# iwa-shi/CRDR

Measured on AMD Instinct MI355X. Metric: stage-3 training img/s at 256x256, higher is better.
Workload: dtype fp32; 1 GPU; config/crdr_stage_3.yaml -b 16: full GAN step (G + 5x CLIC21GVAE D + LPIPS-Alex, random-init weights), rate index cycled 0..4; global_batch=16, crop=256, parallelism=dp1

## Files before the change

crdr_amd/csrc/algo_id.hpp:

```cpp
#pragma once

namespace crdr {

enum AlgoFamily { kAlgoBuiltIn, kAlgoTiled , kAlgoStream, kAlgoWino2, kAlgoWino4, kAlgoBeyond  };
struct AlgoId {
  AlgoFamily family;
  int index;
  int split;
};

inline AlgoId algo_decode(int id, const int (&sizes)[4]) {
  const int base = id & 0xff, split = (id >> 8) & 0xf;
  for (int f = 0, first = 1; id != 0 && f < 4; first += sizes[f++])
    if (base >= first && base < first + sizes[f]) return {AlgoFamily(kAlgoTiled + f), base - first, split};
  return {id == 0 ? kAlgoBuiltIn : kAlgoBeyond, base - 1, split};
}
inline AlgoId conv_algo_decode(int reserved, int ntiled, int nstream) { return algo_decode(reserved, {ntiled, nstream, 2, 1}); }
inline AlgoId wgrad_algo_decode(int algo, int ndirect) { return algo_decode(algo & 0xffff, {ndirect, 0, 1, 1}); }

inline int conv_algo_splits(const AlgoId& id) { return id.family == kAlgoWino4 ? id.split + 1 : 1 << id.split; }
inline int wgrad_algo_splits(const AlgoId& id) { return 1 << id.split; }

inline int conv_algo_encode(AlgoFamily family, int index, int nsplit, int ntiled, int nstream) {
  const int first[] = {1, 1 + ntiled, 1 + ntiled + nstream, 1 + ntiled + nstream + 2};
  int ls = 0;
  while ((1 << ls) < nsplit) ++ls;
  return (first[family - kAlgoTiled] + index) | ((family == kAlgoWino4 ? nsplit - 1 : ls) << 8);
}

}
```

crdr_amd/csrc/api.cpp:

```cpp
#include <hip/hip_runtime.h>
#include <stdarg.h>
#include <stdio.h>

#include <mutex>
#include <vector>

#include "crdr_hip.h"

namespace crdr {
static thread_local char g_err[512] = "";
void set_error(const char* fmt, ...) {
  va_list ap;
  va_start(ap, fmt);
  vsnprintf(g_err, sizeof(g_err), fmt, ap);
  va_end(ap);
}
}

namespace crdr {
struct ProfRec { int kind; double flops; hipEvent_t e0, e1; };
static std::mutex g_pm;
static std::vector<ProfRec> g_recs;
static bool g_prof = false;
bool profile_on() { return g_prof; }
void* profile_begin(hipStream_t s) {
  if (!g_prof) return nullptr;
  hipEvent_t* ev = new hipEvent_t[2];
  if (hipEventCreate(&ev[0]) != hipSuccess || hipEventCreate(&ev[1]) != hipSuccess) { delete[] ev; return nullptr; }
  (void)hipEventRecord(ev[0], s);
  return ev;
}
void profile_end(int kind, double flops, void* token, hipStream_t s) {
  if (!token) return;
  hipEvent_t* ev = static_cast<hipEvent_t*>(token);
  (void)hipEventRecord(ev[1], s);
  std::lock_guard<std::mutex> lk(g_pm);
  g_recs.push_back({kind, flops, ev[0], ev[1]});
  delete[] ev;
}
}

extern "C" void crdr_profile_enable(int on) {
  std::lock_guard<std::mutex> lk(crdr::g_pm);
  crdr::g_prof = on != 0;
}
extern "C" int crdr_profile_read(int kind, double* flops, double* ms, long long* launches) {
  std::lock_guard<std::mutex> lk(crdr::g_pm);
  double f = 0, t = 0;
  long long n = 0;
  std::vector<crdr::ProfRec> keep;
  for (auto& r : crdr::g_recs) {
    if (r.kind != kind) { keep.push_back(r); continue; }
    (void)hipEventSynchronize(r.e1);
    float dt = 0.f;
    if (hipEventElapsedTime(&dt, r.e0, r.e1) == hipSuccess) { f += r.flops; t += dt; ++n; }
    (void)hipEventDestroy(r.e0);
    (void)hipEventDestroy(r.e1);
  }
  crdr::g_recs.swap(keep);
  if (flops) *flops = f;
  if (ms) *ms = t;
  if (launches) *launches = n;
  return 0;
}

extern "C" const char* crdr_last_error(void) { return crdr::g_err; }
extern "C" int crdr_version(void) { return 600; }
extern "C" const char* crdr_arch(void) { return "gfx950"; }
```

crdr_amd/csrc/igemm.hip:

```cpp
#include <algorithm>
#include <type_traits>

#include "algo_id.hpp"
#include "igemm_kernel.hpp"
#include "wino.hpp"

namespace crdr {

extern template __global__ void igemm_kernel<4, 1, 1, 1, false, 0, false>(const IgemmArgs, const IgemmTaps, const IgemmGroup);
extern template __global__ void igemm_kernel<4, 1, 1, 2, false, 0, false>(const IgemmArgs, const IgemmTaps, const IgemmGroup);
extern template __global__ void igemm_kernel<4, 1, 1, 3, false, 0, false>(const IgemmArgs, const IgemmTaps, const IgemmGroup);
extern template __global__ void igemm_kernel<4, 1, 1, 4, false, 0, false>(const IgemmArgs, const IgemmTaps, const IgemmGroup);
extern template __global__ void igemm_kernel<4, 1, 1, 5, false, 0, false>(const IgemmArgs, const IgemmTaps, const IgemmGroup);
extern template __global__ void igemm_kernel<4, 1, 1, 6, false, 0, false>(const IgemmArgs, const IgemmTaps, const IgemmGroup);
extern template __global__ void igemm_kernel<4, 1, 1, 7, false, 0, false>(const IgemmArgs, const IgemmTaps, const IgemmGroup);
extern template __global__ void igemm_kernel<4, 1, 2, 2, false, 0, false>(const IgemmArgs, const IgemmTaps, const IgemmGroup);
extern template __global__ void igemm_kernel<4, 1, 2, 3, false, 0, false>(const IgemmArgs, const IgemmTaps, const IgemmGroup);
extern template __global__ void igemm_kernel<4, 1, 2, 4, false, 0, false>(const IgemmArgs, const IgemmTaps, const IgemmGroup);
extern template __global__ void igemm_kernel<2, 2, 2, 2, false, 0, false>(const IgemmArgs, const IgemmTaps, const IgemmGroup);
extern template __global__ void igemm_kernel<2, 2, 1, 1, false, 0, false>(const IgemmArgs, const IgemmTaps, const IgemmGroup);
extern template __global__ void igemm_kernel<2, 2, 1, 2, false, 0, false>(const IgemmArgs, const IgemmTaps, const IgemmGroup);
extern template __global__ void igemm_kernel<2, 2, 1, 3, false, 0, false>(const IgemmArgs, const IgemmTaps, const IgemmGroup);
extern template __global__ void igemm_kernel<2, 2, 1, 4, false, 0, false>(const IgemmArgs, const IgemmTaps, const IgemmGroup);
extern template __global__ void igemm_kernel<1, 4, 1, 1, false, 0, false>(const IgemmArgs, const IgemmTaps, const IgemmGroup);
extern template __global__ void igemm_kernel<1, 4, 1, 2, false, 0, false>(const IgemmArgs, const IgemmTaps, const IgemmGroup);
extern template __global__ void igemm_kernel<4, 2, 1, 1, false, 0, false>(const IgemmArgs, const IgemmTaps, const IgemmGroup);
extern template __global__ void igemm_kernel<4, 2, 1, 2, false, 0, false>(const IgemmArgs, const IgemmTaps, const IgemmGroup);
extern template __global__ void igemm_kernel<4, 2, 1, 3, false, 0, false>(const IgemmArgs, const IgemmTaps, const IgemmGroup);
extern template __global__ void igemm_kernel<4, 2, 2, 1, false, 0, false>(const IgemmArgs, const IgemmTaps, const IgemmGroup);
extern template __global__ void igemm_kernel<4, 2, 2, 2, false, 0, false>(const IgemmArgs, const IgemmTaps, const IgemmGroup);
extern template __global__ void igemm_kernel<2, 4, 1, 1, false, 0, false>(const IgemmArgs, const IgemmTaps, const IgemmGroup);
extern template __global__ void igemm_kernel<2, 4, 2, 1, false, 0, false>(const IgemmArgs, const IgemmTaps, const IgemmGroup);
extern template __global__ void igemm_kernel<2, 4, 1, 2, false, 0, false>(const IgemmArgs, const IgemmTaps, const IgemmGroup);
extern template __global__ void igemm_kernel<2, 2, 2, 1, false, 0, false>(const IgemmArgs, const IgemmTaps, const IgemmGroup);
extern template __global__ void igemm_kernel<2, 2, 2, 3, false, 0, false>(const IgemmArgs, const IgemmTaps, const IgemmGroup);
extern template __global__ void igemm_kernel<4, 1, 1, 1, true, 0, false>(const IgemmArgs, const IgemmTaps, const IgemmGroup);
extern template __global__ void igemm_kernel<4, 1, 1, 2, true, 0, false>(const IgemmArgs, const IgemmTaps, const IgemmGroup);
extern template __global__ void igemm_kernel<4, 1, 2, 2, true, 0, false>(const IgemmArgs, const IgemmTaps, const IgemmGroup);
extern template __global__ void igemm_kernel<2, 2, 2, 2, true, 0, false>(const IgemmArgs, const IgemmTaps, const IgemmGroup);
extern template __global__ void igemm_kernel<4, 2, 1, 1, true, 0, false>(const IgemmArgs, const IgemmTaps, const IgemmGroup);
extern template __global__ void igemm_kernel<4, 2, 1, 2, true, 0, false>(const IgemmArgs, const IgemmTaps, const IgemmGroup);
extern template __global__ void igemm_kernel<4, 2, 2, 1, true, 0, false>(const IgemmArgs, const IgemmTaps, const IgemmGroup);
extern template __global__ void igemm_kernel<4, 2, 2, 2, true, 0, false>(const IgemmArgs, const IgemmTaps, const IgemmGroup);
extern template __global__ void igemm_kernel<2, 4, 2, 1, true, 0, false>(const IgemmArgs, const IgemmTaps, const IgemmGroup);
extern template __global__ void igemm_kernel<4, 1, 1, 1, false, 3, false>(const IgemmArgs, const IgemmTaps, const IgemmGroup);
extern template __global__ void igemm_kernel<4, 1, 1, 2, false, 3, false>(const IgemmArgs, const IgemmTaps, const IgemmGroup);
extern template __global__ void igemm_kernel<4, 1, 1, 3, false, 3, false>(const IgemmArgs, const IgemmTaps, const IgemmGroup);
extern template __global__ void igemm_kernel<4, 1, 1, 4, false, 3, false>(const IgemmArgs, const IgemmTaps, const IgemmGroup);
extern template __global__ void igemm_kernel<4, 1, 1, 5, false, 3, false>(const IgemmArgs, const IgemmTaps, const IgemmGroup);
extern template __global__ void igemm_kernel<4, 1, 1, 6, false, 3, false>(const IgemmArgs, const IgemmTaps, const IgemmGroup);
extern template __global__ void igemm_kernel<4, 1, 1, 7, false, 3, false>(const IgemmArgs, const IgemmTaps, const IgemmGroup);
extern template __global__ void igemm_kernel<4, 1, 2, 2, false, 3, false>(const IgemmArgs, const IgemmTaps, const IgemmGroup);
extern template __global__ void igemm_kernel<4, 1, 2, 3, false, 3, false>(const IgemmArgs, const IgemmTaps, const IgemmGroup);
extern template __global__ void igemm_kernel<4, 1, 2, 4, false, 3, false>(const IgemmArgs, const IgemmTaps, const IgemmGroup);
extern template __global__ void igemm_kernel<2, 2, 2, 2, false, 3, false>(const IgemmArgs, const IgemmTaps, const IgemmGroup);
extern template __global__ void igemm_kernel<2, 2, 1, 1, false, 3, false>(const IgemmArgs, const IgemmTaps, const IgemmGroup);
extern template __global__ void igemm_kernel<2, 2, 1, 2, false, 3, false>(const IgemmArgs, const IgemmTaps, const IgemmGroup);
extern template __global__ void igemm_kernel<2, 2, 1, 3, false, 3, false>(const IgemmArgs, const IgemmTaps, const IgemmGroup);
extern template __global__ void igemm_kernel<2, 2, 1, 4, false, 3, false>(const IgemmArgs, const IgemmTaps, const IgemmGroup);
extern template __global__ void igemm_kernel<1, 4, 1, 1, false, 3, false>(const IgemmArgs, const IgemmTaps, const IgemmGroup);
extern template __global__ void igemm_kernel<1, 4, 1, 2, false, 3, false>(const IgemmArgs, const IgemmTaps, const IgemmGroup);
extern template __global__ void igemm_kernel<4, 2, 1, 1, false, 3, false>(const IgemmArgs, const IgemmTaps, const IgemmGroup);
extern template __global__ void igemm_kernel<4, 2, 1, 2, false, 3, false>(const IgemmArgs, const IgemmTaps, const IgemmGroup);
extern template __global__ void igemm_kernel<4, 2, 1, 3, false, 3, false>(const IgemmArgs, const IgemmTaps, const IgemmGroup);
extern template __global__ void igemm_kernel<4, 2, 2, 1, false, 3, false>(const IgemmArgs, const IgemmTaps, const IgemmGroup);
extern template __global__ void igemm_kernel<4, 2, 2, 2, false, 3, false>(const IgemmArgs, const IgemmTaps, const IgemmGroup);
extern template __global__ void igemm_kernel<2, 4, 1, 1, false, 3, false>(const IgemmArgs, const IgemmTaps, const IgemmGroup);
extern template __global__ void igemm_kernel<2, 4, 2, 1, false, 3, false>(const IgemmArgs, const IgemmTaps, const IgemmGroup);
extern template __global__ void igemm_kernel<2, 4, 1, 2, false, 3, false>(const IgemmArgs, const IgemmTaps, const IgemmGroup);
extern template __global__ void igemm_kernel<2, 2, 2, 1, false, 3, false>(const IgemmArgs, const IgemmTaps, const IgemmGroup);
extern template __global__ void igemm_kernel<2, 2, 2, 3, false, 3, false>(const IgemmArgs, const IgemmTaps, const IgemmGroup);
extern template __global__ void igemm_kernel<4, 1, 1, 2, false, 6, false>(const IgemmArgs, const IgemmTaps, const IgemmGroup);
extern template __global__ void igemm_kernel<4, 1, 1, 4, false, 6, false>(const IgemmArgs, const IgemmTaps, const IgemmGroup);
extern template __global__ void igemm_kernel<2, 2, 2, 2, false, 6, false>(const IgemmArgs, const IgemmTaps, const IgemmGroup);
extern template __global__ void igemm_kernel<2, 2, 1, 1, false, 6, false>(const IgemmArgs, const IgemmTaps, const IgemmGroup);
extern template __global__ void igemm_kernel<2, 2, 1, 2, false, 6, false>(const IgemmArgs, const IgemmTaps, const IgemmGroup);
extern template __global__ void igemm_kernel<2, 2, 1, 3, false, 6, false>(const IgemmArgs, const IgemmTaps, const IgemmGroup);
extern template __global__ void igemm_kernel<4, 2, 1, 2, false, 6, false>(const IgemmArgs, const IgemmTaps, const IgemmGroup);
extern template __global__ void igemm_kernel<2, 4, 2, 1, false, 6, false>(const IgemmArgs, const IgemmTaps, const IgemmGroup);
extern template __global__ void igemm_kernel<2, 2, 2, 1, false, 6, false>(const IgemmArgs, const IgemmTaps, const IgemmGroup);
extern template __global__ void igemm_kernel<4, 1, 1, 1, false, 0, true>(const IgemmArgs, const IgemmTaps, const IgemmGroup);
extern template __global__ void igemm_kernel<4, 1, 1, 2, false, 0, true>(const IgemmArgs, const IgemmTaps, const IgemmGroup);
extern template __global__ void igemm_kernel<4, 1, 1, 3, false, 0, true>(const IgemmArgs, const IgemmTaps, const IgemmGroup);
extern template __global__ void igemm_kernel<4, 1, 1, 4, false, 0, true>(const IgemmArgs, const IgemmTaps, const IgemmGroup);
extern template __global__ void igemm_kernel<4, 1, 1, 5, false, 0, true>(const IgemmArgs, const IgemmTaps, const IgemmGroup);
extern template __global__ void igemm_kernel<4, 1, 1, 6, false, 0, true>(const IgemmArgs, const IgemmTaps, const IgemmGroup);
extern template __global__ void igemm_kernel<4, 1, 1, 7, false, 0, true>(const IgemmArgs, const IgemmTaps, const IgemmGroup);
extern template __global__ void igemm_kernel<4, 1, 2, 2, false, 0, true>(const IgemmArgs, const IgemmTaps, const IgemmGroup);
extern template __global__ void igemm_kernel<4, 1, 2, 3, false, 0, true>(const IgemmArgs, const IgemmTaps, const IgemmGroup);
extern template __global__ void igemm_kernel<4, 1, 2, 4, false, 0, true>(const IgemmArgs, const IgemmTaps, const IgemmGroup);
extern template __global__ void igemm_kernel<2, 2, 2, 2, false, 0, true>(const IgemmArgs, const IgemmTaps, const IgemmGroup);
extern template __global__ void igemm_kernel<2, 2, 1, 1, false, 0, true>(const IgemmArgs, const IgemmTaps, const IgemmGroup);
extern template __global__ void igemm_kernel<2, 2, 1, 2, false, 0, true>(const IgemmArgs, const IgemmTaps, const IgemmGroup);
extern template __global__ void igemm_kernel<2, 2, 1, 3, false, 0, true>(const IgemmArgs, const IgemmTaps, const IgemmGroup);
extern template __global__ void igemm_kernel<2, 2, 1, 4, false, 0, true>(const IgemmArgs, const IgemmTaps, const IgemmGroup);
extern template __global__ void igemm_kernel<1, 4, 1, 1, false, 0, true>(const IgemmArgs, const IgemmTaps, const IgemmGroup);
extern template __global__ void igemm_kernel<1, 4, 1, 2, false, 0, true>(const IgemmArgs, const IgemmTaps, const IgemmGroup);
extern template __global__ void igemm_kernel<4, 2, 1, 1, false, 0, true>(const IgemmArgs, const IgemmTaps, const IgemmGroup);
extern template __global__ void igemm_kernel<4, 2, 1, 2, false, 0, true>(const IgemmArgs, const IgemmTaps, const IgemmGroup);
extern template __global__ void igemm_kernel<4, 2, 1, 3, false, 0, true>(const IgemmArgs, const IgemmTaps, const IgemmGroup);
extern template __global__ void igemm_kernel<4, 2, 2, 1, false, 0, true>(const IgemmArgs, const IgemmTaps, const IgemmGroup);
extern template __global__ void igemm_kernel<4, 2, 2, 2, false, 0, true>(const IgemmArgs, const IgemmTaps, const IgemmGroup);
extern template __global__ void igemm_kernel<2, 4, 1, 1, false, 0, true>(const IgemmArgs, const IgemmTaps, const IgemmGroup);
extern template __global__ void igemm_kernel<2, 4, 2, 1, false, 0, true>(const IgemmArgs, const IgemmTaps, const IgemmGroup);
extern template __global__ void igemm_kernel<2, 4, 1, 2, false, 0, true>(const IgemmArgs, const IgemmTaps, const IgemmGroup);
extern template __global__ void igemm_kernel<2, 2, 2, 1, false, 0, true>(const IgemmArgs, const IgemmTaps, const IgemmGroup);
extern template __global__ void igemm_kernel<2, 2, 2, 3, false, 0, true>(const IgemmArgs, const IgemmTaps, const IgemmGroup);

using IgemmKern = void (*)(const IgemmArgs, const IgemmTaps, const IgemmGroup);
enum TileForm {
  kPlain,
  kTapMajor,
  kBf3,
  kFast,
  kBf6,
  kNumTileForms
};
struct TileCfg {
  int wm, wn, mb, nb;
  IgemmKern kern[kNumTileForms];
};
static constexpr size_t cfg_lds(int wm, int wn, int mb, int nb, int prec) {
  const size_t BM = 32 * wm * mb, BN = 32 * wn * nb;
  const size_t staging = igemm_staging_floats((int)BM, (int)BN, prec);
  const size_t epi = (size_t)wm * wn * 32 * 32 * (nb < 4 ? nb : 4) + (size_t)wm * 2 * BN;
  const size_t sv_off = ((staging > epi ? staging : epi) + 3) & ~(size_t)3;
  return (sv_off + (size_t)4 * BN + 4) * sizeof(float);
}
template <int a, int b, int c, int d, bool FITS = igemm_bf6_ok(a, b, c, d) && (cfg_lds(a, b, c, d, 6) <= 160 * 1024)>
struct Bf6Kern { static constexpr IgemmKern fn = igemm_kernel<a, b, c, d, false, 6>; };
template <int a, int b, int c, int d>
struct Bf6Kern<a, b, c, d, false> { static constexpr IgemmKern fn = nullptr; };
#define CFG(a, b, c, d) {a, b, c, d, {igemm_kernel<a, b, c, d, false, 0>, nullptr, igemm_kernel<a, b, c, d, false, 3>, igemm_kernel<a, b, c, d, false, 0, true>, Bf6Kern<a, b, c, d>::fn}}
#define CFGS(a, b, c, d) {a, b, c, d, {igemm_kernel<a, b, c, d, false, 0>, igemm_kernel<a, b, c, d, true, 0>, igemm_kernel<a, b, c, d, false, 3>, igemm_kernel<a, b, c, d, false, 0, true>, Bf6Kern<a, b, c, d>::fn}}
static const TileCfg kCfgs[] = {
    CFGS(4, 1, 1, 1), CFGS(4, 1, 1, 2), CFG(4, 1, 1, 3), CFG(4, 1, 1, 4), CFG(4, 1, 1, 5), CFG(4, 1, 1, 6),
    CFG(4, 1, 1, 7),
    CFGS(4, 1, 2, 2), CFG(4, 1, 2, 3), CFG(4, 1, 2, 4),
    CFGS(2, 2, 2, 2),
    CFG(2, 2, 1, 1),
    CFG(2, 2, 1, 2),
    CFG(2, 2, 1, 3),
    CFG(2, 2, 1, 4),
    CFG(1, 4, 1, 1),
    CFG(1, 4, 1, 2),
    CFGS(4, 2, 1, 1),
    CFGS(4, 2, 1, 2),
    CFG(4, 2, 1, 3),
    CFGS(4, 2, 2, 1),
    CFGS(4, 2, 2, 2),
    CFG(2, 4, 1, 1),
    CFGS(2, 4, 2, 1),
    CFG(2, 4, 1, 2),
    CFG(2, 2, 2, 1),
    CFG(2, 2, 2, 3),
};
#undef CFG
#undef CFGS
static const int kNumCfgs = sizeof(kCfgs) / sizeof(kCfgs[0]);

struct Plan {
  IgemmArgs a;
  IgemmTaps t;
  int cfg;
  int stream;
  WinoKernel wino;
  StreamArgs sa;
  dim3 grid;
  size_t lds;
  size_t ws_bytes;
};

static bool splitk_ok(long long tiles, int M, int ws_ld, int ns) {
  return tiles <= CRDR_CONV_TICKETS && (long long)ns * M * ws_ld * 4 < (1ll << 31) - (1 << 24);
}

static int floordiv(int a, int b) {
  int q = a / b, r = a % b;
  return (r != 0 && ((r < 0) != (b < 0))) ? q - 1 : q;
}

static const float kCfgTflops[] = {107, 120, 122, 120, 105, 99, 94, 90, 101, 106, 102, 116, 123, 120, 107, 109, 111, 115, 126, 121,
                                   111, 116, 119, 127, 114, 119, 108};
static_assert(sizeof(kCfgTflops) / sizeof(kCfgTflops[0]) == sizeof(kCfgs) / sizeof(kCfgs[0]), "one figure per configuration");

static void fill_taps(const crdr_conv_desc* d, IgemmArgs& a, IgemmTaps& tp) {
  auto pack_tap = [](int dh, int dw, int widx) { return (dh & 0xff) | ((dw & 0xff) << 8) | (widx << 16); };
  const int S = d->stride, P = d->pad;
  int nt = 0;
  if (!d->transposed) {
    a.nphase = 1; a.GH = d->OH; a.GW = d->OW; a.so = 1; a.si = S;
    tp.poh[0] = 0; tp.pow[0] = 0; tp.tap_begin[0] = 0;
    for (int r = 0; r < d->kh; ++r)
      for (int s = 0; s < d->kw; ++s) {
        tp.packed[nt++] = pack_tap(r - P, s - P, r * d->kw + s);
      }
    tp.tap_begin[1] = (short)nt;
  } else {
    a.nphase = S * S; a.GH = cdiv(d->OH, S); a.GW = cdiv(d->OW, S); a.so = S; a.si = 1;
    int ph = 0;
    for (int py = 0; py < S; ++py)
      for (int px = 0; px < S; ++px, ++ph) {
        tp.poh[ph] = (int8_t)py; tp.pow[ph] = (int8_t)px; tp.tap_begin[ph] = (short)nt;
        for (int r = 0; r < d->kh; ++r) {
          if (((py + P - r) % S + S) % S) continue;
          for (int s = 0; s < d->kw; ++s) {
            if (((px + P - s) % S + S) % S) continue;
            tp.packed[nt++] = pack_tap(floordiv(py + P - r, S), floordiv(px + P - s, S), r * d->kw + s);
          }
        }
      }
    tp.tap_begin[ph] = (short)nt;
  }
}

static int plan_geometry(const crdr_conv_desc* d, Plan* pl, int G) {
  IgemmArgs& a = pl->a;
  IgemmTaps& tp = pl->t;
  memset(&a, 0, sizeof(a));
  memset(&tp, 0, sizeof(tp));
  CRDR_REQUIRE(d->kh * d->kw <= 128, "conv2d: kernel %dx%d has more than 128 taps", d->kh, d->kw);
  CRDR_REQUIRE(d->stride >= 1 && d->stride <= 4, "conv2d: stride %d unsupported", d->stride);
  CRDR_REQUIRE(d->C % 4 == 0 && d->ldx % 4 == 0, "conv2d: C (%d) and ldx (%d) must be multiples of 4", d->C, d->ldx);
  CRDR_REQUIRE(d->wcols % 32 == 0 && d->wcols >= d->C && d->wrows >= d->OC, "conv2d: bad weight pack %dx%d", d->wrows,
               d->wcols);
  a.N = d->N; a.H = d->H; a.W = d->W; a.Cin = d->C; a.ldx = d->ldx;
  a.OH = d->OH; a.OW = d->OW; a.ldy = d->ldy; a.Cout = d->OC;
  a.wrows = d->wrows; a.wcols = d->wcols;
  a.ldres = d->ldres; a.ldg = d->ldg; a.flags = d->flags;
  a.ldpre = d->ldpre; a.ldmask = d->ldmask; a.ngroup = G;
  CRDR_REQUIRE(G >= 1 && G <= CRDR_MAX_GROUP, "conv2d: group of %d problems (max %d)", G, CRDR_MAX_GROUP);
  a.smallc = d->wlayout == 1;
  CRDR_REQUIRE(!a.smallc || (!d->transposed && d->C <= 4 && d->wcols >= 4 * d->kh * d->kw),
               "conv2d: tap-major weight layout needs a non-transposed conv with C <= 4 and wcols >= 4*taps");
  a.kchunks = a.smallc ? cdiv(d->kh * d->kw, 8) : cdiv(d->C, 32);
  fill_taps(d, a, tp);
  {
    const long long hw = (long long)a.GH * a.GW;
    const bool p2 = a.GW > 0 && hw > 0 && hw < (1ll << 30) && (a.GW & (a.GW - 1)) == 0 && (hw & (hw - 1)) == 0;
    a.gw_sh = p2 ? __builtin_ctz((unsigned)a.GW) : -1;
    a.hw_sh = p2 ? __builtin_ctzll((unsigned long long)hw) : -1;
  }
  {
    const long long xb = (((long long)d->N * d->H * d->W - 1) * d->ldx + d->C) * 4;
    const long long wb = (long long)(a.smallc ? 1 : d->kh * d->kw) * d->wrows * d->wcols * 4;
    CRDR_REQUIRE(wb < (1ll << 31), "conv2d: weight pack (%lld B) reaches 2 GiB", wb);
    CRDR_REQUIRE((long long)d->W * d->ldx * 4 * (d->kh + 2) < (1ll << 30), "conv2d: an image row (%d px x %d floats) is too wide", d->W, d->ldx);
    a.x_bytes = (unsigned long long)xb;
    a.w_bytes = (unsigned)wb;
  }
  const long long M64 = (long long)d->N * a.GH * a.GW;
  CRDR_REQUIRE(M64 < (1ll << 31) && (long long)d->N * d->H * d->W < (1ll << 31), "conv2d: too many pixels");
  a.M = (int)M64;
  CRDR_REQUIRE(!((d->flags & CRDR_CONV_BF16X6) && (d->flags & CRDR_CONV_BF16X3)), "conv2d: CRDR_CONV_BF16X3 and CRDR_CONV_BF16X6 are exclusive");
  a.cs_ld = round_up(d->OC, 32);
  a.nsplit = 1;
  pl->cfg = pl->stream = -1;
  pl->wino = WinoKernel::None;
  pl->grid = dim3(1, 1, 1);
  pl->lds = pl->ws_bytes = 0;
  return 0;
}

static int plan_wino(const crdr_conv_desc* d, Plan* pl, int G, const AlgoId& id, bool fallback) {
  const bool f4 = id.family == kAlgoWino4;
  int nsplit = 1;
  if (f4) {
    CRDR_REQUIRE(!fallback && wino4_eligible(d, G, true), "conv2d: forced F(4x4, 3x3) Winograd kernel: not a 3x3 / 5x5 stride-1 or 5x5 stride-2 convolution it takes (wino4_eligible)");
    nsplit = conv_algo_splits(id);
    CRDR_REQUIRE(wino4_split_ok(d, G, nsplit), "conv2d: F(4x4, 3x3) Winograd kernel: %d K splits do not fit this shape", nsplit);
  } else {
    CRDR_REQUIRE(!fallback && wino_eligible(d, G), "conv2d: forced Winograd kernel: not a 3x3 / 5x5 stride-1 convolution it takes");
    CRDR_REQUIRE(id.index == 0 || wino_pairs_ok(d), "conv2d: Winograd pair-tile variant: needs a channel tail of 1..32 and more than one patch");
    CRDR_REQUIRE(id.split == 0, "conv2d: the Winograd kernel has no split-K");
  }
  pl->wino = f4 ? WinoKernel::F4 : (id.index == 1 ? WinoKernel::F2Pairs : WinoKernel::F2);
  pl->a.nsplit = nsplit;
  if (d->flags & CRDR_EPI_COLSUM) pl->a.cs_rows = f4 ? wino4_colsum_rows(d) : wino_colsum_rows(d);
  pl->ws_bytes = (size_t)CRDR_CONV_TICKETS * sizeof(int) + (f4 ? wino4_workspace(d, G, nsplit) : wino_workspace(d, G));
  return 0;
}

static int choose_stream(const crdr_conv_desc* d, const IgemmArgs& a, int G) {
  if ((d->flags & CRDR_EPI_COLSUM) || (long long)a.M * G < 16384 || d->ldy % 4 != 0 || ((d->flags & CRDR_EPI_RES) && d->ldres % 4 != 0) ||
      ((d->flags & (CRDR_EPI_RELUMASK | CRDR_EPI_LRELUMASK)) && d->ldmask % 4 != 0))
    return -1;
  static const int pref[] = {1, 2, 0, 3};
  long long bestpad = 1ll << 60;
  int best = -1;
  for (int q = 0; q < 4; ++q) {
    const int sv = 4 + pref[q];
    size_t lds;
    if (sv >= stream_num_variants() || stream_fits(d, sv, &lds) != StreamFit::kOk) continue;
    int snb, sst, snw;
    stream_variant_shape(sv, &snb, &sst, &snw);
    const long long pad = (long long)cdiv(d->OC, 32 * snb) * (32 * snb);
    if (pad < bestpad) { bestpad = pad; best = sv; }
  }
  return best;
}

static int plan_stream(const crdr_conv_desc* d, Plan* pl, int G, int sv, int forced_split) {
  IgemmArgs& a = pl->a;
  CRDR_REQUIRE(forced_split == 0, "conv2d: the streaming 1x1 kernel has no split-K");
  size_t lds = 0;
  const StreamFit fit = stream_fits(d, sv, &lds);
  CRDR_REQUIRE(fit != StreamFit::kShape,
               "conv2d: the streaming kernel takes 1x1 stride-1 convolutions with C %% 32 == 0, OC %% 4 == 0 and no "
               "gate / pre-add / accumulate epilogue");
  int snb, sstages, snw;
  stream_variant_shape(sv, &snb, &sstages, &snw);
  const int BN = 32 * snb, SBM = 32 * snw;
  CRDR_REQUIRE(fit != StreamFit::kLds, "conv2d: streaming variant %d needs %zu B of LDS for C = %d", sv, lds, d->C);
  const int gridN = cdiv(d->OC, BN), mtiles = cdiv(a.M, SBM);
  CRDR_REQUIRE(fit != StreamFit::kColumnTiles, "conv2d: streaming variant %d: %d column tiles", sv, gridN);
  const int nlanes = std::max(8, std::min(256 / (gridN * G) / 8 * 8, round_up(mtiles, 8)));
  pl->stream = sv;
  pl->sa.gridN = gridN;
  pl->sa.nlanes = nlanes;
  pl->grid = dim3(G * gridN * nlanes, 1, 1);
  pl->lds = lds;
  if (d->flags & CRDR_EPI_COLSUM) a.cs_rows = mtiles;
  return 0;
}

static void choose_tile(const crdr_conv_desc* d, const IgemmArgs& a, int KT, int G, int max_split, int* bc, int* bs) {
  double best = 1e300;
  const bool bf6 = (d->flags & CRDR_CONV_BF16X6) && !a.smallc;
  for (int c = 0; c < kNumCfgs; ++c) {
    const TileCfg& t = kCfgs[c];
    if (a.smallc && !t.kern[kTapMajor]) continue;
    if (bf6 && !t.kern[kBf6]) continue;
    const int BM = 32 * t.wm * t.mb, BN = 32 * t.wn * t.nb;
    const long long tiles = (long long)cdiv(a.M, BM) * cdiv(d->OC, BN) * a.nphase;
    for (int ns = 1; ns <= max_split; ns *= 2) {
      if (ns > 1 && KT / ns < 4) break;
      if (ns > 1 && !splitk_ok(tiles * G, a.M, cdiv(d->OC, BN) * BN, ns)) break;
      const long long blocks = tiles * ns * G;
      const double per_iter = 16.0 * t.mb * t.nb * 64.0 * std::max(1.0, t.wm * t.wn / 4.0) * (133.0 / kCfgTflops[c]) *
                              ((d->flags & CRDR_CONV_BF16X3) && !a.smallc ? 0.3 : (bf6 ? 0.5 : 1.0));
      const double waves = (double)cdiv64(blocks, 256);
      double cost = waves * ((double)cdiv(KT, ns) * per_iter + 3000.0);
      if (ns > 1) cost += 7000.0 + (double)BM * BN * ns * 4.0 / 40.0;
      if (cost < best) { best = cost; *bc = c; *bs = ns; }
    }
  }
}

static int plan_tiled(const crdr_conv_desc* d, Plan* pl, int G, const AlgoId& id, bool fallback) {
  IgemmArgs& a = pl->a;
  int maxtaps = 0;
  for (int ph = 0; ph < a.nphase; ++ph) maxtaps = std::max(maxtaps, (int)(pl->t.tap_begin[ph + 1] - pl->t.tap_begin[ph]));
  const int KT = a.smallc ? a.kchunks : maxtaps * a.kchunks;
  const bool bf6 = (d->flags & CRDR_CONV_BF16X6) && !a.smallc;
  int bc = -1, bs = 1;
  if (id.family == kAlgoBuiltIn) {
    choose_tile(d, a, KT, G, (fallback || (d->flags & CRDR_CONV_NOSPLIT)) ? 1 : 16, &bc, &bs);
  } else {
    bc = id.index;
    bs = conv_algo_splits(id);
    CRDR_REQUIRE(id.family == kAlgoTiled, "conv2d: forced config %d out of range", bc);
    CRDR_REQUIRE(!a.smallc || kCfgs[bc].kern[kTapMajor], "conv2d: config %d has no tap-major variant", bc);
    CRDR_REQUIRE(!bf6 || kCfgs[bc].kern[kBf6], "conv2d: config %d has no bf16x6 variant (its stages do not fit LDS)", bc);
    CRDR_REQUIRE(bs == 1 || KT / bs >= 2, "conv2d: forced split %d too deep for %d K-iterations", bs, KT);
    CRDR_REQUIRE(bs == 1 || !(d->flags & CRDR_CONV_NOSPLIT), "conv2d: forced split %d with CRDR_CONV_NOSPLIT", bs);
    if (bs > 1) {
      const TileCfg& ft = kCfgs[bc];
      const int fBM = 32 * ft.wm * ft.mb, fBN = 32 * ft.wn * ft.nb;
      CRDR_REQUIRE(splitk_ok((long long)cdiv(a.M, fBM) * cdiv(d->OC, fBN) * a.nphase * G, a.M, cdiv(d->OC, fBN) * fBN, bs),
                   "conv2d: forced split %d: too many tiles or slabs too large for the in-launch reduce", bs);
    }
  }
  CRDR_REQUIRE(bc >= 0, "conv2d: no tile config");
  const TileCfg& t = kCfgs[bc];
  const int BM = 32 * t.wm * t.mb, BN = 32 * t.wn * t.nb;
  pl->cfg = bc;
  a.nsplit = bs;
  pl->grid = dim3(cdiv(a.M, BM), cdiv(d->OC, BN), a.nphase * bs * G);
  {
    const double A = (double)d->N * d->H * d->W * d->C * 4.0, B = (double)a.w_bytes;
    a.m_inner = (G == 1 && B >= 32.0e6 && A * 4.0 <= B) ? 1 : 0;
  }
  a.ws_ld = pl->grid.y * BN;
  {
    static const int mode = [] { const char* e = getenv("CRDR_K_CMAJOR"); return e ? atoi(e) : -1; }();
    const bool applies = !a.smallc && maxtaps > 1 && a.kchunks > 1;
    a.k_cmajor = applies && (mode == 1 || (mode < 0 && d->C >= 1024)) ? 1 : 0;
  }
  pl->lds = cfg_lds(t.wm, t.wn, t.mb, t.nb, bf6 ? 6 : 0);
  if (d->flags & CRDR_EPI_COLSUM) a.cs_rows = a.nphase * (int)pl->grid.x;
  pl->ws_bytes = bs > 1 ? (size_t)CRDR_CONV_TICKETS * sizeof(int) + (size_t)G * a.nphase * bs * a.M * a.ws_ld * sizeof(float) : 0;
  return 0;
}

static int build_plan(const crdr_conv_desc* d, Plan* pl, int G = 1, bool fallback = false) {
  if (int rc = plan_geometry(d, pl, G)) return rc;
  const AlgoId id = conv_algo_decode(d->reserved, kNumCfgs, stream_num_variants());
  if (id.family == kAlgoWino2 || id.family == kAlgoWino4) return plan_wino(d, pl, G, id, fallback);
  int sv = id.family == kAlgoStream ? id.index : -1;
  if (id.family == kAlgoBuiltIn && !fallback) sv = choose_stream(d, pl->a, G);
  if (sv >= 0) return plan_stream(d, pl, G, sv, id.split);
  return plan_tiled(d, pl, G, id, fallback);
}

}

using namespace crdr;

extern "C" int crdr_conv2d_num_configs(void) { return kNumCfgs; }
extern "C" int crdr_conv2d_num_stream_configs(void) { return stream_num_variants(); }
extern "C" int crdr_conv2d_num_wino_configs(void) { return 3; }

extern "C" size_t crdr_conv2d_grouped_workspace(const crdr_conv_desc* d, int G) {
  Plan pl;
  return build_plan(d, &pl, G) ? 0 : pl.ws_bytes;
}
extern "C" size_t crdr_conv2d_workspace(const crdr_conv_desc* d) { return crdr_conv2d_grouped_workspace(d, 1); }

extern "C" int crdr_conv2d_colsum_layout(const crdr_conv_desc* d, int G, int* rows, int* ld) {
  CRDR_REQUIRE(d && rows && ld, "conv2d_colsum_layout: null pointer");
  Plan pl;
  if (int rc = build_plan(d, &pl, G)) return rc;
  *rows = pl.a.cs_rows;
  *ld = pl.a.cs_ld;
  return 0;
}

extern "C" int crdr_conv2d_choose_algo(const crdr_conv_desc* d, int G) {
  Plan pl;
  if (!d || build_plan(d, &pl, G)) return 0;
  const bool f4 = pl.wino == WinoKernel::F4, f2 = pl.wino == WinoKernel::F2 || pl.wino == WinoKernel::F2Pairs;
  const AlgoFamily family = f4 ? kAlgoWino4 : (f2 ? kAlgoWino2 : (pl.stream >= 0 ? kAlgoStream : kAlgoTiled));
  const int index = f4 ? 0 : (f2 ? (pl.wino == WinoKernel::F2Pairs ? 1 : 0) : (pl.stream >= 0 ? pl.stream : pl.cfg));
  return conv_algo_encode(family, index, pl.a.nsplit, kNumCfgs, stream_num_variants());
}

extern "C" double crdr_conv2d_flops(const crdr_conv_desc* d) {
  if (!d->transposed) return 2.0 * d->N * d->OH * d->OW * (double)d->OC * d->C * d->kh * d->kw;
  return 2.0 * d->N * d->H * d->W * (double)d->OC * d->C * d->kh * d->kw;
}

static bool al16(const void* q) { return (reinterpret_cast<uintptr_t>(q) & 15) == 0; }

static int check_io(const crdr_conv_desc* d, const crdr_conv_io* ios, int G, size_t need_ws, size_t ws_bytes) {
  const crdr_conv_io& io = ios[0];
  const int flags = d->flags;
  CRDR_REQUIRE(!(flags & CRDR_EPI_VEC2) || io.vec2, "conv2d: VEC2 flag without vec2");
  CRDR_REQUIRE(!(flags & CRDR_EPI_RES) || io.res, "conv2d: RES flag without res");
  CRDR_REQUIRE(!((flags & CRDR_EPI_RELUMASK) && (flags & CRDR_EPI_LRELUMASK)), "conv2d: RELUMASK and LRELUMASK are exclusive");
  CRDR_REQUIRE(!(flags & CRDR_EPI_AFFINE) || (io.scale && io.shift), "conv2d: AFFINE flag without scale/shift");
  CRDR_REQUIRE(!(flags & CRDR_EPI_GATE) || (io.gx && io.gt && io.sig), "conv2d: GATE flag without gx/gt/sig");
  CRDR_REQUIRE(G == 1 || !(flags & (CRDR_EPI_VEC2 | CRDR_EPI_AFFINE | CRDR_EPI_GATE | CRDR_EPI_MASKOFF)),
               "conv2d_grouped: epilogue flags %d not supported in a grouped launch", flags);
  CRDR_REQUIRE(!(flags & CRDR_EPI_MASKOFF) || ((flags & (CRDR_EPI_RELUMASK | CRDR_EPI_LRELUMASK)) && io.vec2 && !(flags & CRDR_EPI_VEC2)),
               "conv2d: MASKOFF needs a mask flag and vec2, and excludes VEC2");
  CRDR_REQUIRE(need_ws <= ws_bytes, "conv2d: workspace too small (%zu < %zu)", ws_bytes, need_ws);
  for (int g = 0; g < G; ++g) {
    const crdr_conv_io& q = ios[g];
    CRDR_REQUIRE(q.x && q.w && q.y, "conv2d: null tensor (problem %d)", g);
    CRDR_REQUIRE(al16(q.x) && al16(q.w), "conv2d: x and w must be 16-byte aligned (problem %d)", g);
    CRDR_REQUIRE(!(flags & CRDR_EPI_BIAS) || q.bias, "conv2d: BIAS flag without bias (problem %d)", g);
    CRDR_REQUIRE(!(flags & CRDR_EPI_PREADD) || q.pre, "conv2d: PREADD flag without pre (problem %d)", g);
    CRDR_REQUIRE(!(flags & (CRDR_EPI_RELUMASK | CRDR_EPI_LRELUMASK)) || q.mask, "conv2d: mask flag without mask (problem %d)", g);
    CRDR_REQUIRE(!(flags & CRDR_EPI_RES) || q.res, "conv2d: RES flag without res (problem %d)", g);
    CRDR_REQUIRE(!(flags & CRDR_EPI_COLSUM) || q.cs, "conv2d: COLSUM flag without cs (problem %d)", g);
  }
  return 0;
}

static bool rows_aligned(const crdr_conv_desc* d, const crdr_conv_io* ios, int G) {
  const bool res = d->flags & CRDR_EPI_RES, gate = d->flags & CRDR_EPI_GATE, pre = d->flags & CRDR_EPI_PREADD;
  const bool mask = d->flags & (CRDR_EPI_RELUMASK | CRDR_EPI_LRELUMASK);
  bool v = d->ldy % 4 == 0 && (!res || d->ldres % 4 == 0) && (!pre || d->ldpre % 4 == 0) && (!mask || d->ldmask % 4 == 0) &&
           (!gate || (d->ldg % 4 == 0 && al16(ios[0].gx) && al16(ios[0].gt) && al16(ios[0].sig)));
  for (int g = 0; g < G; ++g) {
    const crdr_conv_io& q = ios[g];
    v = v && al16(q.y) && (!res || al16(q.res)) && (!pre || al16(q.pre)) && (!mask || al16(q.mask));
  }
  return v;
}

static bool fast_epilogue_ok(const IgemmArgs& a, bool vec_epi) {
  const long long span_px = (256 / std::max(a.GW, 1) + 2) * (long long)std::max(a.so, 1) * a.OW + a.OW;
  const long long span = span_px * std::max(std::max(a.ldy, a.ldres), a.ldmask) * 4;
  return vec_epi && a.Cout % 4 == 0 && span < (1ll << 31) && !(a.flags & (CRDR_EPI_GATE | CRDR_EPI_PREADD | CRDR_EPI_ACCUM));
}

static void bind_io(Plan* pl, const crdr_conv_io* ios, int G, void* ws, IgemmGroup* grp) {
  IgemmArgs& a = pl->a;
  const crdr_conv_io& io = ios[0];
  a.x = io.x; a.w = io.w; a.y = io.y;
  a.counters = (int*)ws;
  a.ws = (float*)ws + CRDR_CONV_TICKETS;
  a.bias = io.bias; a.vec2 = io.vec2; a.res = io.res; a.scale = io.scale; a.shift = io.shift;
  a.gx = io.gx; a.gt = io.gt; a.sig = io.sig; a.pre = io.pre; a.mask = io.mask; a.cs = io.cs;
  memset(grp, 0, sizeof(*grp));
  for (int g = 0; g < G; ++g) {
    const crdr_conv_io& q = ios[g];
    grp->x[g] = q.x; grp->w[g] = q.w; grp->y[g] = q.y; grp->bias[g] = q.bias; grp->pre[g] = q.pre; grp->mask[g] = q.mask;
    grp->res[g] = q.res; grp->cs[g] = q.cs;
  }
}

static int launch_conv(const crdr_conv_desc* d, const crdr_conv_io* ios, int G, void* ws, size_t ws_bytes, crdr_stream_t s,
                       float* ucache = nullptr, size_t ucache_bytes = 0, int ucache_valid = 0) {
  Plan pl;
  if (int rc = build_plan(d, &pl, G)) return rc;
  if (pl.a.M == 0) return 0;
  if (int rc = check_io(d, ios, G, pl.ws_bytes, ws_bytes)) return rc;
  const bool vec_epi = rows_aligned(d, ios, G);
  if (pl.stream >= 0 && !vec_epi && d->reserved == 0) {
    if (int rc = build_plan(d, &pl, G, true)) return rc;
  }
  IgemmGroup grp;
  bind_io(&pl, ios, G, ws, &grp);
  IgemmArgs& a = pl.a;
  a.vec_epi = vec_epi ? 1 : 0;
  a.fast_epi = fast_epilogue_ok(a, vec_epi) ? 1 : 0;
  if (pl.wino != WinoKernel::None) {
    const bool f4 = pl.wino == WinoKernel::F4;
    void* prof = profile_begin(as_stream(s));
    if (f4) {
      const size_t u_bytes = wino4_workspace(d, G, 1);
      float* u = (float*)ws + CRDR_CONV_TICKETS;
      if (ucache) {
        CRDR_REQUIRE(ucache_bytes >= u_bytes, "conv2d: filter cache of %zu bytes, the launch needs %zu", ucache_bytes, u_bytes);
        u = ucache;
      }
      float* slabs = (float*)ws + CRDR_CONV_TICKETS + u_bytes / 4;
      if (int rc = wino4_launch(d, a, pl.t, grp, G, u, slabs, a.nsplit, ucache && ucache_valid, as_stream(s))) return rc;
    } else if (int rc = wino_launch(d, pl.wino == WinoKernel::F2Pairs, a, pl.t, grp, G, (float*)ws + CRDR_CONV_TICKETS, as_stream(s))) return rc;
    profile_end(f4 ? (d->kh == 5 ? 6 : 5) : 3, G * crdr_conv2d_flops(d), prof, as_stream(s));
    return 0;
  }
  if (pl.stream >= 0) {
    CRDR_REQUIRE(a.vec_epi, "conv2d: the streaming kernel needs 16-byte aligned operand rows");
    void* prof = profile_begin(as_stream(s));
    stream_launch(pl.stream, a, pl.sa, grp, pl.grid.x, pl.lds, as_stream(s));
    CRDR_CHECK_LAUNCH("gemm1x1_kernel");
    profile_end(0, G * crdr_conv2d_flops(d), prof, as_stream(s));
    return 0;
  }
  const TileCfg& t = kCfgs[pl.cfg];
  const TileForm form = a.smallc ? kTapMajor : ((d->flags & CRDR_CONV_BF16X3) ? kBf3 : ((d->flags & CRDR_CONV_BF16X6) ? kBf6 : ((a.fast_epi && a.nsplit == 1) ? kFast : kPlain)));
  const IgemmKern kern = t.kern[form];
  CRDR_REQUIRE(kern, "conv2d: config %d has no kernel for this precision", pl.cfg);
  static std::atomic<bool> attr_done[kNumTileForms][64];
  allow_full_lds(attr_done[form][pl.cfg], kern);
  void* prof = profile_begin(as_stream(s));
  hipLaunchKernelGGL(kern, pl.grid, dim3(64 * t.wm * t.wn), pl.lds, as_stream(s), a, pl.t, grp);
  CRDR_CHECK_LAUNCH("igemm_kernel");
  profile_end(0, G * crdr_conv2d_flops(d), prof, as_stream(s));
  return 0;
}

extern "C" int crdr_conv2d(const crdr_conv_desc* d, const crdr_conv_io* io, void* ws, size_t ws_bytes,
                           crdr_stream_t s) {
  CRDR_REQUIRE(d && io, "conv2d: null descriptor");
  return launch_conv(d, io, 1, ws, ws_bytes, s);
}

extern "C" int crdr_conv2d_grouped(const crdr_conv_desc* d, const crdr_conv_io* ios, int G, void* ws, size_t ws_bytes,
                                   crdr_stream_t s) {
  CRDR_REQUIRE(d && ios, "conv2d_grouped: null descriptor");
  CRDR_REQUIRE(G >= 1 && G <= CRDR_MAX_GROUP, "conv2d_grouped: %d problems (1..%d)", G, CRDR_MAX_GROUP);
  return launch_conv(d, ios, G, ws, ws_bytes, s);
}

extern "C" size_t crdr_conv2d_filter_cache_bytes(const crdr_conv_desc* d, int G) {
  Plan pl;
  if (!d || G < 1 || G > CRDR_MAX_GROUP || build_plan(d, &pl, G) || pl.wino != WinoKernel::F4) return 0;
  return wino4_workspace(d, G, 1);
}

extern "C" int crdr_conv2d_filter_item(const crdr_conv_desc* d, int G, crdr_w4_filter_item* item) {
  CRDR_REQUIRE(d && item, "conv2d_filter_item: null pointer");
  CRDR_REQUIRE(G >= 1 && G <= CRDR_MAX_GROUP, "conv2d_filter_item: %d problems (1..%d)", G, CRDR_MAX_GROUP);
  Plan pl;
  if (int rc = build_plan(d, &pl, G)) return rc;
  CRDR_REQUIRE(pl.wino == WinoKernel::F4, "conv2d_filter_item: the descriptor's `reserved` does not force the F(4x4, 3x3) kernel");
  return wino4_filter_item(d, pl.t, G, item);
}

extern "C" int crdr_w4_filters_batched(const crdr_w4_filter_item* items, const int64_t* prefix, const int64_t* meta, crdr_stream_t s) {
  CRDR_REQUIRE(items && prefix && meta, "w4_filters_batched: null pointer");
  return wino4_filters_batched(items, reinterpret_cast<const long long*>(prefix), reinterpret_cast<const long long*>(meta), as_stream(s));
}

extern "C" int crdr_conv2d_grouped_ex(const crdr_conv_desc* d, const crdr_conv_io* ios, int G, void* ws, size_t ws_bytes, float* filter_cache,
                                      size_t filter_cache_bytes, int filter_cache_valid, crdr_stream_t s) {
  CRDR_REQUIRE(d && ios, "conv2d_grouped_ex: null descriptor");
  CRDR_REQUIRE(G >= 1 && G <= CRDR_MAX_GROUP, "conv2d_grouped_ex: %d problems (1..%d)", G, CRDR_MAX_GROUP);
  CRDR_REQUIRE(!filter_cache || (reinterpret_cast<uintptr_t>(filter_cache) & 15) == 0, "conv2d_grouped_ex: the filter cache must be 16-byte aligned");
  return launch_conv(d, ios, G, ws, ws_bytes, s, filter_cache, filter_cache_bytes, filter_cache_valid);
}
```

crdr_amd/csrc/wino.hpp:

```cpp
#pragma once
#include <algorithm>

#include "common.hpp"
#include "igemm_args.hpp"

namespace crdr {

inline int tap_window(const IgemmTaps& taps, int k, const char* who, bool complete, int* win, int* dmin) {
  *dmin = 127;
  for (int t = 0; t < k * k; ++t) *dmin = std::min(*dmin, (int)(signed char)(taps.packed[t] & 0xff));
  for (int t = 0; t < k * k; ++t) win[t] = -1;
  for (int t = 0; t < k * k; ++t) {
    const int v = taps.packed[t];
    const int dh = (int)(signed char)(v & 0xff) - *dmin, dw = (int)(signed char)((v >> 8) & 0xff) - *dmin;
    CRDR_REQUIRE(dh >= 0 && dh < k && dw >= 0 && dw < k, "conv2d: %s: tap offsets are not a %dx%d window", who, k, k);
    win[dh * k + dw] = v >> 16;
  }
  for (int t = 0; complete && t < k * k; ++t) CRDR_REQUIRE(win[t] >= 0, "conv2d: %s: incomplete %dx%d window", who, k, k);
  return 0;
}

inline bool wino_admits(const crdr_conv_desc* d, int G) {
  if (d->flags & (CRDR_EPI_GATE | CRDR_EPI_PREADD | CRDR_CONV_BF16X3)) return false;
  if (G > 1 && (d->flags & (CRDR_EPI_VEC2 | CRDR_EPI_AFFINE | CRDR_EPI_MASKOFF))) return false;
  return ((long long)d->N * d->H + 8) * d->W * d->ldx * 4 < (1ll << 31);
}

enum class WinoKernel { None, F2, F2Pairs, F4 };

bool wino_eligible(const crdr_conv_desc* d, int G);
size_t wino_workspace(const crdr_conv_desc* d, int G);
int wino_colsum_rows(const crdr_conv_desc* d);
bool wino_pairs_ok(const crdr_conv_desc* d);
int wino_launch(const crdr_conv_desc* d, bool pairs, IgemmArgs a, const IgemmTaps& taps, const IgemmGroup& grp, int G, float* u, hipStream_t s);

bool wino4_eligible(const crdr_conv_desc* d, int G, bool vec_ok);
size_t wino4_workspace(const crdr_conv_desc* d, int G, int nsplit);
bool wino4_split_ok(const crdr_conv_desc* d, int G, int nsplit);
int wino4_colsum_rows(const crdr_conv_desc* d);
int wino4_filter_item(const crdr_conv_desc* d, const IgemmTaps& taps, int G, crdr_w4_filter_item* it);
int wino4_filters_batched(const crdr_w4_filter_item* items, const long long* prefix, const long long* meta, hipStream_t s);
int wino4_launch(const crdr_conv_desc* d, IgemmArgs a, const IgemmTaps& taps, const IgemmGroup& grp, int G, float* u, float* slabs, int nsplit,
                 bool filters_ready, hipStream_t s);

}
```

crdr_amd/csrc/wino4.hip:

```cpp
#include <algorithm>
#include <type_traits>

#include "common.hpp"
#include "igemm_args.hpp"
#include "wino.hpp"
#include "wino4_xform.hpp"

namespace crdr {

namespace {

constexpr int kNT4 = 256;

template <int GEO> struct W4Geo {
  static constexpr int TY = GEO == 0 ? 2 : 4, TX = GEO == 0 ? 16 : (GEO == 1 ? 8 : 4), PR = TX + 1, USED = GEO == 2 ? 57 : (TY + 1) * (TX + 1);
};
template <int GEO> __device__ __forceinline__ int w4_ty(int th, int tx) { return GEO == 0 ? th : (GEO == 1 ? 2 * th + (tx >> 3) : tx >> 2); }
template <int GEO> __device__ __forceinline__ int w4_tx(int tx) { return GEO == 0 ? tx : (GEO == 1 ? tx & 7 : tx & 3); }
template <int GEO> __device__ __forceinline__ int w4_slot0(int th) { return GEO == 2 ? 32 * th : 0; }
constexpr int kBN4 = 64;
constexpr int kClsSlots = 64;
constexpr int kInUsed4 = 16 * kClsSlots;
constexpr int kInPieces = 16;
constexpr int kInSlots4 = kInPieces * 64;
constexpr int kUSlots4 = 36 * 4 * kBN4 / 4;
constexpr int kRawBufs = 3, kFiltBufs = 3;
constexpr int kRF = kInSlots4 * 4, kFF = kUSlots4 * 4;
constexpr int kLdsFloats4 = kRawBufs * kRF + kFiltBufs * kFF;

__device__ __forceinline__ void lds_barrier4() {
  __builtin_amdgcn_sched_barrier(0);
  __builtin_amdgcn_s_waitcnt(0xC07F);
  __builtin_amdgcn_s_barrier();
  __builtin_amdgcn_sched_barrier(0);
}

__device__ __forceinline__ void at6_pk(const f32x2v m0, const f32x2v m1, const f32x2v m2, const f32x2v m3, const f32x2v m4, const f32x2v m5,
                                       f32x2v& o0, f32x2v& o1, f32x2v& o2, f32x2v& o3) {
  const f32x2v p = m1 + m2, q = m1 - m2, u = m3 + m4, w = m3 - m4;
  o0 = m0 + p + u;
  o1 = pk_fma(pk_bc(kWb), w, pk_bc(kWa) * q);
  o2 = pk_fma(pk_bc(kWb2), u, pk_bc(kWa2) * p);
  o3 = pk_fma(pk_bc(kWb3), w, pk_bc(kWa3) * q) + m5;
}

struct Wino4Tile { int gidx, n, oh0, ow0, n0, patch, tn, phase, lin, ks, kbeg, kcnt; };

template <int GEO>
__device__ __forceinline__ Wino4Tile wino4_tile(const IgemmArgs& p, int vb, int gx, int gyn_, int gz) {
  const bool fstat = gyn_ < 0;
  const int gyn = fstat ? -gyn_ : gyn_;
  Wino4Tile t;
  const int nph = p.so * p.so;
  const int T = gx * gyn * nph, S = p.nsplit, nwg = T * gz * S, cpx = nwg >> 3;
  const int qs = vb < cpx * 8 ? (vb & 7) * cpx + (vb >> 3) : vb;
  const int q = qs / S;
  t.ks = qs - q * S;
  t.lin = q;
  {
    const int cnt = (p.kchunks + S - 1) / S;
    t.kbeg = t.ks * cnt;
    t.kcnt = min(cnt, p.kchunks - t.kbeg);
  }
  t.gidx = q / T;
  const int r = q - t.gidx * T;
  int tn;
  if (fstat) {
    const int combo = r / gx;
    t.patch = r - combo * gx;
    tn = combo / nph;
    t.phase = combo - tn * nph;
  } else {
    t.phase = r % nph;
    const int r1 = r / nph;
    tn = r1 % gyn;
    t.patch = r1 / gyn;
  }
  t.tn = tn;
  if constexpr (GEO == 2) {
    t.n = 2 * t.patch;
    t.oh0 = 0;
    t.ow0 = 0;
  } else {
    const int ppi = p.GH * p.GW;
    t.n = t.patch / ppi;
    const int prem = t.patch - t.n * ppi, by = prem / p.GW, bx = prem - by * p.GW;
    t.oh0 = by * (4 * W4Geo<GEO>::TY);
    t.ow0 = bx * (4 * W4Geo<GEO>::TX);
  }
  t.n0 = tn * kBN4;
  return t;
}

template <int GEO>
__device__ __forceinline__ unsigned wino4_piece_geo(int piece, int lane) {
  using G = W4Geo<GEO>;
  const int S = piece * 64 + lane;
  const int cls = S / kClsSlots, r2f = S - cls * kClsSlots;
  const int img = GEO == 2 ? r2f >> 5 : 0, r2 = GEO == 2 ? r2f & 31 : r2f;
  const int R = r2 / G::PR, Cc = r2 - R * G::PR;
  const int ci = cls >> 2, cj = cls & 3;
  const bool used = S < kInUsed4 && r2 < (GEO == 2 ? 25 : G::USED);
  return (unsigned)(4 * R + ci) | ((unsigned)(4 * Cc + cj) << 8) | ((unsigned)img << 16) | ((used ? 1u : 0u) << 17);
}
template <int GEO, int FORM>
__device__ __forceinline__ unsigned wino4_in_off(const IgemmArgs& p, const Wino4Tile& t, unsigned geo, int sub) {
  using G = W4Geo<GEO>;
  const int pi = (int)(geo & 0xff) + (FORM == 1 ? 3 * (sub >> 1) : 0), pj = (int)((geo >> 8) & 0xff) + (FORM == 1 ? 3 * (sub & 1) : 0);
  const int pmax_i = 4 * G::TY + 2 + (FORM == 1 ? 3 * (sub >> 1) : 0), pmax_j = 4 * G::TX + 2 + (FORM == 1 ? 3 * (sub & 1) : 0);
  const int n = t.n + (int)((geo >> 16) & 1);
  const int ist = (FORM == 0 && p.nphase == 4) ? 2 : 1;
  const int ih = ist * (t.oh0 - p.si + pi), iw = ist * (t.ow0 - p.si + pj);
  const bool ok = ((geo >> 17) & 1) && pi < pmax_i && pj < pmax_j && n < p.N && (unsigned)ih < (unsigned)p.H && (unsigned)iw < (unsigned)p.W;
  return ok ? (unsigned)((((n * p.H + ih) * p.W + iw) * p.ldx) * 4) : kOobOffset;
}

struct Wino4Src {
  __amdgpu_buffer_rsrc_t rx, ru;
  unsigned u_off0;
  unsigned a_off[4];
};

__device__ __forceinline__ __amdgpu_buffer_rsrc_t wino4_empty_rsrc() { return __builtin_amdgcn_make_buffer_rsrc(nullptr, 0, 0, 0x00020000); }

__device__ __forceinline__ void wino4_dma_raw(float* smem, const Wino4Src& sr, __amdgpu_buffer_rsrc_t rx, int j, int soff, int rbuf, int lane, int wave) {
  const int piece = wave + 4 * j;
  __builtin_amdgcn_raw_ptr_buffer_load_lds(rx, (lds_ptr_t)(smem + rbuf * kRF + piece * 256), 16, (int)sr.a_off[j], soff, 0, 0);
}
template <int FORM>
__device__ __forceinline__ int wino4_raw_soff(const IgemmArgs& p, int kr) {
  if (p.nphase == 1) return kr * 16;
  const int Kc = p.kchunks / p.nphase, sub = kr / Kc, ch = kr - sub * Kc;
  if (FORM == 1) return ch * 16;
  return ch * 16 + ((sub >> 1) * p.W + (sub & 1)) * p.ldx * 4;
}
__device__ __forceinline__ void wino4_dma_filt(float* smem, const Wino4Src& sr, __amdgpu_buffer_rsrc_t ru, int j, int kf, int fbuf, int lane, int wave) {
  const int piece = wave * 9 + j;
  const unsigned so = (unsigned)__builtin_amdgcn_readfirstlane((int)sr.u_off0) + (unsigned)kf * (kUSlots4 * 16u) + (unsigned)piece * 1024u;
  __builtin_amdgcn_raw_ptr_buffer_load_lds(ru, (lds_ptr_t)(smem + kRawBufs * kRF + fbuf * kFF + piece * 256), 16, lane * 16, (int)so, 0, 0);
}
constexpr int kW4PrologueReqs = 30;
template <int FORM>
__device__ __forceinline__ void wino4_prologue_req(const IgemmArgs& p, float* smem, const Wino4Src& sr, int kbeg, int kcnt, int lane, int wave, int i) {
  if (i < 12) {
    const int kr = i >> 2;
    wino4_dma_raw(smem, sr, kr < kcnt ? sr.rx : wino4_empty_rsrc(), i & 3, wino4_raw_soff<FORM>(p, kbeg + kr), kr, lane, wave);
  } else {
    const int kf = (i - 12) / 9;
    wino4_dma_filt(smem, sr, kf < kcnt ? sr.ru : wino4_empty_rsrc(), (i - 12) - 9 * kf, kbeg + kf, kf, lane, wave);
  }
}
template <int FORM>
__device__ __forceinline__ void wino4_prologue_dma(const IgemmArgs& p, float* smem, const Wino4Src& sr, int kbeg, int kcnt, int lane, int wave) {
#pragma unroll
  for (int i = 0; i < kW4PrologueReqs; ++i) wino4_prologue_req<FORM>(p, smem, sr, kbeg, kcnt, lane, wave, i);
}
struct Wino4Next { bool more; int kbeg, kcnt; };

template <int GEO, int FORM>
__device__ __forceinline__ void wino4_loop(const IgemmArgs& p, const Wino4Tile& tl, float* smem, Wino4Src& sr, bool prefetched, int lane, int wave,
                                           f32x4 (&acc)[64], f32x4 (&accv)[8], const unsigned (&geo)[4]) {
  const int K4 = tl.kcnt, kbeg = tl.kbeg;
  const int tx = lane & 15, kg = lane >> 4, th = wave >> 1, oh = wave & 1;
  const int rbase = (w4_slot0<GEO>(th) + w4_ty<GEO>(th, tx) * W4Geo<GEO>::PR + w4_tx<GEO>(tx)) * 4 + kg;
  auto ro = [](int i, int j) constexpr { return (((i & 3) * 4 + (j & 3)) * kClsSlots + (i >> 2) * W4Geo<GEO>::PR + (j >> 2)) * 4; };
  const int fbase = kRawBufs * kRF + kg * kBN4 + 32 * oh + 2 * tx;

  const W4Consts kc = w4_consts();
  f32x2v T[6][3];
  f32x2v V[6][3];
  f32x2v D[2][6];
  auto vread = [&](const float* rp, int r) __attribute__((always_inline)) {
    const int c = r / 6, i = r - 6 * c;
    D[c & 1][i] = f32x2v{rp[ro(i, 2 * c)], rp[ro(i, 2 * c + 1)]};
  };
  auto vpass = [&](int c) __attribute__((always_inline)) {
    f32x2v t6[6];
    bt6_cols(D[c & 1], t6, kc);
#pragma unroll
    for (int xi = 0; xi < 6; ++xi) T[xi][c] = t6[xi];
  };
  auto hpass = [&](int x) __attribute__((always_inline)) { bt6_row(T[x][0], T[x][1], T[x][2], V[x], kc); };

  if (!prefetched) {
    wino4_prologue_dma<FORM>(p, smem, sr, kbeg, K4, lane, wave);
    __builtin_amdgcn_s_waitcnt(0x0070);
  } else {
    __builtin_amdgcn_s_waitcnt(0x8070);
  }
  lds_barrier4();
  {
    const float* rp = smem + rbase;
#pragma unroll
    for (int c = 0; c < 3; ++c) {
#pragma unroll
      for (int i = 0; i < 6; ++i) vread(rp, 6 * c + i);
      vpass(c);
    }
#pragma unroll
    for (int x = 0; x < 5; ++x) hpass(x);
  }

  float uf[9][2];
#pragma unroll
  for (int j = 0; j < 4; ++j) {
    const f32x2 u2 = *reinterpret_cast<const f32x2*>(smem + fbase + j * 256);
    uf[j][0] = u2[0];
    uf[j][1] = u2[1];
  }
  int r1 = 1, r0 = 0;
  const int Kc = p.kchunks / p.nphase;
  int ch3 = (kbeg + 3) % Kc, sub3 = (kbeg + 3) / Kc;
  if constexpr (FORM == 1) {
    if (sub3 != kbeg / Kc && sub3 < 4) {
#pragma unroll
      for (int j = 0; j < 4; ++j) sr.a_off[j] = wino4_in_off<GEO, FORM>(p, tl, geo[j], sub3);
    }
  }
  struct SubState {
    int rpo, fpo, fpno;
    __amdgpu_buffer_rsrc_t ru2, rx3;
    int soff3, f2;
  };
  auto sub_state = [&](int k, int r0_, int r1_, int ch3_, int sub3_) __attribute__((always_inline)) {
    SubState st;
    st.rpo = rbase + r1_ * kRF;
    st.fpo = fbase + r0_ * kFF;
    st.fpno = fbase + r1_ * kFF;
    asm volatile("" : "+v"(st.rpo));
    asm volatile("" : "+v"(st.fpo));
    asm volatile("" : "+v"(st.fpno));
    st.ru2 = k + 2 < K4 ? sr.ru : wino4_empty_rsrc();
    st.rx3 = k + 3 < K4 ? sr.rx : wino4_empty_rsrc();
    st.soff3 = FORM == 1 ? ch3_ * 16 : ch3_ * 16 + ((sub3_ >> 1) * p.W + (sub3_ & 1)) * p.ldx * 4;
    st.f2 = r1_ == 2 ? 0 : r1_ + 1;
    return st;
  };
  SubState cur = sub_state(0, r0, r1, ch3, sub3), nxt = cur;
  for (int k = 0; k < K4; ++k) {
    const float* rp = smem + cur.rpo;
    const float* fp = smem + cur.fpo;
    const __amdgpu_buffer_rsrc_t ru2 = cur.ru2, rx3 = cur.rx3;
    const int soff3 = cur.soff3, f2 = cur.f2;
    const float* fpn = smem + cur.fpno;
    bool newsub = false;
    hpass(5);
    __builtin_amdgcn_sched_barrier(0);
#pragma clang loop unroll(full)
    for (int s = 0; s < 72; ++s) {
      const int j = s >> 1, ob = s & 1, x = j / 6, y = j - 6 * x;
      if (s < 64) acc[s] = __builtin_amdgcn_mfma_f32_16x16x4f32(uf[j % 9][ob], v_elem(V[x], y), acc[s], 0, 0, 0);
      else asm volatile("v_mfma_f32_16x16x4_f32 %0, %1, %2, %0" : "+v"(accv[s - 64]) : "v"(uf[j % 9][ob]), "v"(v_elem(V[x], y)));
      if (ob == 1 && j + 4 < 36) {
        const f32x2 u2 = *reinterpret_cast<const f32x2*>(fp + (j + 4) * 256);
        uf[(j + 4) % 9][0] = u2[0];
        uf[(j + 4) % 9][1] = u2[1];
      }
      if (s == 70) {
        r0 = r1;
        r1 = r1 == 2 ? 0 : r1 + 1;
        if (++ch3 == Kc) {
          ch3 = 0;
          ++sub3;
          newsub = true;
        }
        nxt = sub_state(k + 1, r0, r1, ch3, sub3);
      }
      if (s >= 66 && s < 70) {
        const f32x2 u2 = *reinterpret_cast<const f32x2*>(fpn + (s - 66) * 256);
        uf[s - 66][0] = u2[0];
        uf[s - 66][1] = u2[1];
      }
      if (ob == 0 && s < 36) vread(rp, s >> 1);
      if (ob == 0 && s >= 36 && s <= 60) {
        const int q = (s - 36) >> 1;
        if (q < 9) wino4_dma_filt(smem, sr, ru2, q, kbeg + k + 2, f2, lane, wave);
        else wino4_dma_raw(smem, sr, rx3, q - 9, soff3, r0, lane, wave);
      }
      __builtin_amdgcn_sched_barrier(0);
      if (s == 15) vpass(0);
      if (s == 27) vpass(1);
      if (s == 39) vpass(2);
      if (s == 41) hpass(0);
      if (s == 44) hpass(1);
      if (s == 47) hpass(2);
      if (s == 50) hpass(3);
      if (s == 62) hpass(4);
      if (s == 15 || s == 27 || s == 39 || s == 41 || s == 44 || s == 47 || s == 50 || s == 62) __builtin_amdgcn_sched_barrier(0);
      if (s == 65) {
        __builtin_amdgcn_s_waitcnt(0x007D);
        __builtin_amdgcn_s_barrier();
        __builtin_amdgcn_sched_barrier(0);
      }
    }
    cur = nxt;
    if constexpr (FORM == 1) {
      if (newsub && sub3 < 4) {
#pragma unroll
        for (int j = 0; j < 4; ++j) sr.a_off[j] = wino4_in_off<GEO, FORM>(p, tl, geo[j], sub3);
      }
    }
    __builtin_amdgcn_sched_barrier(0);
  }
}

__device__ __forceinline__ float acc_read(float v) {
  float o;
  asm volatile("v_accvgpr_read_b32 %0, %1" : "=v"(o) : "a"(v));
  return o;
}

constexpr int kW4EpiA = CRDR_EPI_BIAS | CRDR_EPI_RELU | CRDR_EPI_LRELU | CRDR_EPI_VEC2 | CRDR_EPI_AFFINE;
constexpr int kW4EpiC = CRDR_EPI_BIAS | CRDR_EPI_RELUMASK | CRDR_EPI_LRELUMASK | CRDR_EPI_MASKOFF | CRDR_EPI_COLSUM | CRDR_EPI_ACCUM;
constexpr int kW4EpiAll = kW4EpiA | kW4EpiC | CRDR_EPI_RES;
constexpr int w4_epi_mask(int cls) { return cls == 0 ? kW4EpiA : cls == 1 ? (kW4EpiA | CRDR_EPI_RES) : cls == 2 ? kW4EpiC : kW4EpiAll; }
constexpr int w4_epi_class(int flags) {
  const int f = flags & kW4EpiAll;
  return (f & ~w4_epi_mask(0)) == 0 ? 0 : (f & ~w4_epi_mask(1)) == 0 ? 1 : (f & ~w4_epi_mask(2)) == 0 ? 2 : 3;
}

template <int GEO, int FORM, bool SPLIT, int FM>
__device__ __forceinline__ void wino4_finish(const IgemmArgs& p, const Wino4Tile& tl, float* smem, const float* sV, int lane, int wave, f32x4 (&acc)[64],
                                             f32x4 (&accv)[8], const Wino4Src& srn, const Wino4Next nx) {
  const int f = p.flags & FM;
  const bool has_res = (f & CRDR_EPI_RES) != 0, has_mask = (f & (CRDR_EPI_RELUMASK | CRDR_EPI_LRELUMASK)) != 0;
  const bool do_cs = (f & CRDR_EPI_COLSUM) != 0, accum = (f & CRDR_EPI_ACCUM) != 0;
  const int tx = lane & 15, kg = lane >> 4, th = wave >> 1, oh = wave & 1;
  const int oy0 = tl.oh0 + 4 * w4_ty<GEO>(th, tx), ox0 = tl.ow0 + 4 * w4_tx<GEO>(tx);
  auto tdesc = [&](const float* base, int ld) __attribute__((always_inline)) {
    const unsigned long long bytes = (((unsigned long long)p.N * p.OH * p.OW - 1) * ld + p.Cout) * 4ull;
    return __builtin_amdgcn_make_buffer_rsrc(const_cast<float*>(base), 0, (unsigned)bytes, 0x00020000);
  };
  const __amdgpu_buffer_rsrc_t ry = tdesc(p.y, p.ldy), rr = tdesc(has_res ? p.res : p.y, p.ldres), rm = tdesc(has_mask ? p.mask : p.y, p.ldmask);
  const int so = p.so, py = tl.phase >> 1, px = tl.phase & 1;
  const int img = tl.n + (GEO == 2 ? th : 0);
  const unsigned pix00 = (unsigned)(((size_t)img * p.OH + so * oy0 + py) * p.OW + so * ox0 + px);
  unsigned pixm = 0;
#pragma unroll
  for (int a = 0; a < 4; ++a)
#pragma unroll
    for (int b = 0; b < 4; ++b) pixm |= (img < p.N && so * (oy0 + a) + py < p.OH && so * (ox0 + b) + px < p.OW) ? (1u << (4 * a + b)) : 0u;
  auto soff = [&](int ld, int a, int b) __attribute__((always_inline)) { return so * (a * p.OW + b) * ld * 4; };
  float* sC = smem + kRawBufs * kRF + 2 * kFF;

  auto next_reqs = [&](int grp) __attribute__((always_inline)) {
    __builtin_amdgcn_sched_barrier(0);
#pragma unroll
    for (int i = (3 * grp) / 2; i < (3 * (grp + 1)) / 2; ++i) wino4_prologue_req<FORM>(p, smem, srn, nx.kbeg, nx.kcnt, lane, wave, i);
    __builtin_amdgcn_sched_barrier(0);
  };
  auto out_transform = [&](int ob, float (&yv)[4][4][4], auto reqs_c) __attribute__((always_inline)) {
    constexpr bool REQS = decltype(reqs_c)::value;
#pragma unroll
    for (int rp = 0; rp < 2; ++rp) {
      f32x2v sv[4][6];
#pragma unroll
      for (int nu = 0; nu < 6; ++nu) {
        if constexpr (REQS) next_reqs(10 * rp + nu);
        f32x2v mcol[6];
#pragma unroll
        for (int xi = 0; xi < 6; ++xi) {
          const int blk = 2 * (xi * 6 + nu) + ob;
#pragma unroll
          for (int e = 0; e < 2; ++e)
            mcol[xi][e] = blk < 64 ? acc_read(acc[blk < 64 ? blk : 0][2 * rp + e]) : accv[blk >= 64 ? blk - 64 : 0][2 * rp + e];
        }
        at6_pk(mcol[0], mcol[1], mcol[2], mcol[3], mcol[4], mcol[5], sv[0][nu], sv[1][nu], sv[2][nu], sv[3][nu]);
      }
#pragma unroll
      for (int a = 0; a < 4; ++a) {
        if constexpr (REQS) next_reqs(10 * rp + 6 + a);
        f32x2v y0, y1, y2, y3;
        at6_pk(sv[a][0], sv[a][1], sv[a][2], sv[a][3], sv[a][4], sv[a][5], y0, y1, y2, y3);
#pragma unroll
        for (int e = 0; e < 2; ++e) {
          yv[a][0][2 * rp + e] = y0[e];
          yv[a][1][2 * rp + e] = y1[e];
          yv[a][2][2 * rp + e] = y2[e];
          yv[a][3][2 * rp + e] = y3[e];
        }
      }
      __builtin_amdgcn_sched_barrier(0);
    }
  };
  __amdgpu_buffer_rsrc_t rws = ry;
  unsigned slab_bytes = 0;
  auto slab_off = [&](int ob, int q) __attribute__((always_inline)) { return (unsigned)((((wave * 2 + ob) * 16 + q) * 64 + lane) * 16); };
  if constexpr (SPLIT) {
    if (nx.more) wino4_prologue_dma<FORM>(p, smem, srn, nx.kbeg, nx.kcnt, lane, wave);
    constexpr unsigned kTileSlab = 4u * 2u * 16u * 64u * 16u;
    slab_bytes = (unsigned)p.ws_ld * kTileSlab;
    rws = __builtin_amdgcn_make_buffer_rsrc(p.ws + (size_t)tl.lin * (kTileSlab / 4), 0, 0x7fffffff, 0x00020000);
#pragma unroll
    for (int ob = 0; ob < 2; ++ob) {
      float yv[4][4][4];
      out_transform(ob, yv, std::false_type{});
#pragma unroll
      for (int q = 0; q < 16; ++q) {
        const f32x4 v = {yv[q >> 2][q & 3][0], yv[q >> 2][q & 3][1], yv[q >> 2][q & 3][2], yv[q >> 2][q & 3][3]};
        __builtin_amdgcn_raw_buffer_store_b128(__builtin_bit_cast(u32x4_t, v), rws, slab_off(ob, q) + (unsigned)tl.ks * slab_bytes, 0, 16 );
      }
    }
    asm volatile("s_waitcnt vmcnt(0)" ::: "memory");
    lds_barrier4();
    int* sFlag = reinterpret_cast<int*>(smem + kLdsFloats4 + 2 * 4 * kBN4);
    if (wave == 0 && lane == 0) {
      int* cnt = p.counters + tl.lin;
      const int ticket = __hip_atomic_fetch_add(cnt, 1, __ATOMIC_RELAXED, __HIP_MEMORY_SCOPE_AGENT);
      const int last = ticket == p.nsplit - 1;
      if (last) {
        __hip_atomic_store(cnt, 0, __ATOMIC_RELAXED, __HIP_MEMORY_SCOPE_AGENT);
        __builtin_amdgcn_fence(__ATOMIC_ACQUIRE, "agent");
        asm volatile("s_waitcnt vmcnt(0)" ::: "memory");
      }
      *sFlag = last;
    }
    lds_barrier4();
    const int last = *sFlag;
    if (!last) return;
  }

#pragma unroll
  for (int ob = 0; ob < 2; ++ob) {
    const int cl = 32 * oh + 16 * ob + 4 * kg;
    const int c0 = tl.n0 + cl;
    const bool c_ok = c0 < p.Cout;
    const unsigned okm = c_ok ? pixm : 0u;
    const unsigned base_y = (pix00 * (unsigned)p.ldy + (unsigned)c0) * 4u, base_r = (pix00 * (unsigned)p.ldres + (unsigned)c0) * 4u,
                   base_m = (pix00 * (unsigned)p.ldmask + (unsigned)c0) * 4u;
    auto voff = [&](unsigned base, int a, int b) __attribute__((always_inline)) { return ((okm >> (4 * a + b)) & 1u) ? base : kOobOffset; };
    const int nopnd = (has_res ? 1 : 0) + (has_mask ? 1 : 0) + (accum ? 1 : 0);
    f32x4 opnd[2][8];
    auto fetch = [&](f32x4 (&dst)[8], __amdgpu_buffer_rsrc_t rs, unsigned base, int ld, int hf) __attribute__((always_inline)) {
#pragma unroll
      for (int q = 0; q < 8; ++q) {
        const int a = 2 * hf + (q >> 2), b = q & 3;
        dst[q] = __builtin_bit_cast(f32x4, __builtin_amdgcn_raw_buffer_load_b128(rs, voff(base, a, b), soff(ld, a, b), 0));
      }
    };
    auto fetch_single = [&](int hf) __attribute__((always_inline)) {
      if (has_res) fetch(opnd[hf], rr, base_r, p.ldres, hf);
      else if (has_mask) fetch(opnd[hf], rm, base_m, p.ldmask, hf);
      else fetch(opnd[hf], ry, base_y, p.ldy, hf);
    };
    if (nopnd == 1) fetch_single(0);
    const f32x4 bias = *reinterpret_cast<const f32x4*>(sV + 0 * kBN4 + cl);
    const f32x4 vec2 = *reinterpret_cast<const f32x4*>(sV + 1 * kBN4 + cl);
    const f32x4 scale = *reinterpret_cast<const f32x4*>(sV + 2 * kBN4 + cl);
    const f32x4 shift = *reinterpret_cast<const f32x4*>(sV + 3 * kBN4 + cl);
    f32x4 cpre = {0.f, 0.f, 0.f, 0.f}, cpost = {0.f, 0.f, 0.f, 0.f};
    float yv[4][4][4];
    if constexpr (SPLIT) {
#pragma unroll
      for (int q = 0; q < 16; ++q) {
        f32x4 v = {0.f, 0.f, 0.f, 0.f};
        for (int s0 = 0; s0 < p.nsplit; s0 += 4) {
          f32x4 l[4];
#pragma unroll
          for (int j = 0; j < 4; ++j)
            l[j] = __builtin_bit_cast(f32x4, __builtin_amdgcn_raw_buffer_load_b128(rws, s0 + j < p.nsplit ? slab_off(ob, q) + (unsigned)(s0 + j) * slab_bytes : kOobOffset, 0, 16));
#pragma unroll
          for (int j = 0; j < 4; ++j) v += l[j];
        }
#pragma unroll
        for (int r = 0; r < 4; ++r) yv[q >> 2][q & 3][r] = v[r];
      }
    } else if (ob == 0 && nx.more) {
      out_transform(ob, yv, std::true_type{});
    } else {
      out_transform(ob, yv, std::false_type{});
    }
#pragma unroll
    for (int hf = 0; hf < 2; ++hf) {
      if (nopnd == 1 && hf == 0) fetch_single(1);
      f32x4 o[8];
      bool pix_ok[8];
#pragma unroll
      for (int q = 0; q < 8; ++q) {
        const int a = 2 * hf + (q >> 2), b = q & 3;
        o[q] = f32x4{yv[a][b][0], yv[a][b][1], yv[a][b][2], yv[a][b][3]};
        pix_ok[q] = ((okm >> (4 * a + b)) & 1u) != 0;
      }
      if (f & CRDR_EPI_BIAS) {
#pragma unroll
        for (int q = 0; q < 8; ++q) o[q] += bias;
      }
      if (f & CRDR_EPI_RELU) {
#pragma unroll
        for (int q = 0; q < 8; ++q)
#pragma unroll
          for (int e = 0; e < 4; ++e) o[q][e] = fmaxf(o[q][e], 0.0f);
      }
      if (f & CRDR_EPI_LRELU) {
#pragma unroll
        for (int q = 0; q < 8; ++q)
#pragma unroll
          for (int e = 0; e < 4; ++e) o[q][e] = o[q][e] > 0.0f ? o[q][e] : 0.2f * o[q][e];
      }
      if (f & CRDR_EPI_VEC2) {
#pragma unroll
        for (int q = 0; q < 8; ++q) o[q] += vec2;
      }
      if (has_res) {
        if (nopnd > 1) fetch(opnd[hf], rr, base_r, p.ldres, hf);
#pragma unroll
        for (int q = 0; q < 8; ++q) o[q] += opnd[hf][q];
      }
      if (f & CRDR_EPI_AFFINE) {
#pragma unroll
        for (int q = 0; q < 8; ++q) o[q] = o[q] * scale + shift;
      }
      if (do_cs) {
#pragma unroll
        for (int q = 0; q < 8; ++q)
#pragma unroll
          for (int e = 0; e < 4; ++e) cpre[e] += pix_ok[q] ? o[q][e] : 0.f;
      }
      if (has_mask) {
        if (nopnd > 1) fetch(opnd[hf], rm, base_m, p.ldmask, hf);
        const f32x4 moff = (f & CRDR_EPI_MASKOFF) ? vec2 : f32x4{0.f, 0.f, 0.f, 0.f};
        if (f & CRDR_EPI_LRELUMASK) {
#pragma unroll
          for (int q = 0; q < 8; ++q)
#pragma unroll
            for (int e = 0; e < 4; ++e) o[q][e] = (opnd[hf][q][e] - moff[e]) > 0.0f ? o[q][e] : 0.2f * o[q][e];
        } else {
#pragma unroll
          for (int q = 0; q < 8; ++q)
#pragma unroll
            for (int e = 0; e < 4; ++e) o[q][e] = (opnd[hf][q][e] - moff[e]) > 0.0f ? o[q][e] : 0.0f;
        }
      }
      if (do_cs) {
#pragma unroll
        for (int q = 0; q < 8; ++q)
#pragma unroll
          for (int e = 0; e < 4; ++e) cpost[e] += pix_ok[q] ? o[q][e] : 0.f;
      }
      if (accum) {
        if (nopnd > 1) fetch(opnd[hf], ry, base_y, p.ldy, hf);
#pragma unroll
        for (int q = 0; q < 8; ++q) o[q] += opnd[hf][q];
      }
#pragma unroll
      for (int q = 0; q < 8; ++q) {
        const int a = 2 * hf + (q >> 2), b = q & 3;
        __builtin_amdgcn_raw_buffer_store_b128(__builtin_bit_cast(u32x4_t, o[q]), ry, voff(base_y, a, b), soff(p.ldy, a, b), 0);
      }
    }
    if (do_cs) {
      *reinterpret_cast<f32x4*>(sC + (((wave * 2 + 0) * 2 + ob) * 64 + lane) * 4) = cpre;
      *reinterpret_cast<f32x4*>(sC + (((wave * 2 + 1) * 2 + ob) * 64 + lane) * 4) = cpost;
    }
  }
  if (do_cs) {
    lds_barrier4();
    const int tid = wave * 64 + lane;
    if (tid < 128) {
      const int which = tid >> 6, c = tid & 63, oh2 = c >> 5, ob2 = (c >> 4) & 1, kg2 = (c >> 2) & 3, r = c & 3;
      float sum = 0.f;
      for (int th2 = 0; th2 < 2; ++th2)
        for (int t2 = 0; t2 < 16; ++t2) sum += sC[((((th2 * 2 + oh2) * 2 + which) * 2 + ob2) * 64 + kg2 * 16 + t2) * 4 + r];
      if (tl.n0 + c < p.Cout) p.cs[(((size_t)tl.patch * (p.so * p.so) + tl.phase) * 2 + which) * p.cs_ld + tl.n0 + c] = sum;
    }
  }
}

template <int GEO, int FORM>
__device__ __forceinline__ Wino4Src wino4_src(const IgemmArgs& p, const IgemmGroup& grp, const Wino4Tile& tl, int gyn, const unsigned (&geo)[4]) {
  Wino4Src sr;
  const float* x = p.ngroup > 1 ? grp.x[tl.gidx] : p.x;
  sr.rx = __builtin_amdgcn_make_buffer_rsrc(const_cast<float*>(x), 0, (unsigned)((((unsigned long long)p.N * p.H * p.W - 1) * p.ldx + p.Cin) * 4ull), 0x00020000);
  const int nph = p.so * p.so;
  const size_t ublock = (size_t)gyn * nph * p.kchunks * kUSlots4 * 4;
  sr.ru = __builtin_amdgcn_make_buffer_rsrc(const_cast<float*>(p.w) + (size_t)tl.gidx * ublock, 0, (unsigned)(ublock * 4), 0x00020000);
  sr.u_off0 = (unsigned)(tl.tn * nph + tl.phase) * (unsigned)p.kchunks * (kUSlots4 * 16u);
  const int sub0 = FORM == 1 ? tl.kbeg / (p.kchunks / p.nphase) : 0;
#pragma unroll
  for (int j = 0; j < 4; ++j) sr.a_off[j] = wino4_in_off<GEO, FORM>(p, tl, geo[j], sub0);
  return sr;
}

struct Wino4Vec { float v[4]; };
__device__ __forceinline__ Wino4Vec wino4_vectors_load(const IgemmArgs& p, const IgemmGroup& grp, const Wino4Tile& tl, int tid) {
  Wino4Vec r = {{0.f, 0.f, 1.f, 0.f}};
  if (tid < kBN4) {
    const int f0 = p.flags;
    const bool live = tl.n0 + tid < p.Cout;
    const float* bias = p.ngroup > 1 ? grp.bias[tl.gidx] : p.bias;
    if (live && (f0 & CRDR_EPI_BIAS)) r.v[0] = bias[tl.n0 + tid];
    if (live && (f0 & (CRDR_EPI_VEC2 | CRDR_EPI_MASKOFF))) r.v[1] = p.vec2[tl.n0 + tid];
    if (live && (f0 & CRDR_EPI_AFFINE)) {
      r.v[2] = p.scale[tl.n0 + tid];
      r.v[3] = p.shift[tl.n0 + tid];
    }
  }
  return r;
}
__device__ __forceinline__ void wino4_vectors_store(const Wino4Vec& r, float* sV, int tid) {
  if (tid < kBN4) {
#pragma unroll
    for (int k = 0; k < 4; ++k) sV[k * kBN4 + tid] = r.v[k];
  }
}

template <int GEO, int FORM, bool SPLIT, int EC>
__global__ __launch_bounds__(kNT4) void wino4_kernel(const IgemmArgs p_, const IgemmGroup grp, int gx, int gyn, int gz) {
  extern __shared__ __attribute__((aligned(16))) float smem[];
  const int lane_ = threadIdx.x & 63, wave_ = __builtin_amdgcn_readfirstlane(threadIdx.x >> 6);
  const int gyn_abs = gyn < 0 ? -gyn : gyn;
  const int total = gx * gyn_abs * gz * p_.so * p_.so * (SPLIT ? p_.nsplit : 1);
  float* sVb = smem + kLdsFloats4;
  int cur = 0;
  bool prefetched = false;
  Wino4Src sr;
  unsigned geo[4];
#pragma unroll
  for (int j = 0; j < 4; ++j) geo[j] = wino4_piece_geo<GEO>(wave_ + 4 * j, lane_);
  for (int vb = blockIdx.x; vb < total; vb += gridDim.x) {
    int lane = lane_, wave = wave_;
    asm volatile("" : "+v"(lane));
    asm volatile("" : "+s"(wave));
    const int tid = wave * 64 + lane;
    const Wino4Tile tl = wino4_tile<GEO>(p_, vb, gx, gyn, gz);
    IgemmArgs p = p_;
    if (p.ngroup > 1) {
      const int g = tl.gidx;
      p.x = grp.x[g]; p.y = grp.y[g]; p.bias = grp.bias[g]; p.mask = grp.mask[g]; p.res = grp.res[g]; p.cs = grp.cs[g];
    }
    float* sV = sVb + cur * (4 * kBN4);
    if (!prefetched) {
      const Wino4Vec vec = wino4_vectors_load(p_, grp, tl, tid);
      sr = wino4_src<GEO, FORM>(p_, grp, tl, gyn_abs, geo);
      wino4_vectors_store(vec, sV, tid);
    }
    f32x4 acc[64], accv[8];
#pragma unroll
    for (int j = 0; j < 64; ++j) acc[j] = f32x4{0.f, 0.f, 0.f, 0.f};
#pragma unroll
    for (int j = 0; j < 8; ++j) accv[j] = f32x4{0.f, 0.f, 0.f, 0.f};
    wino4_loop<GEO, FORM>(p, tl, smem, sr, prefetched, lane, wave, acc, accv, geo);
    const bool more = vb + (int)gridDim.x < total;
    Wino4Next nx{false, 0, 0};
    if (more) {
      const Wino4Tile tn = wino4_tile<GEO>(p_, vb + (int)gridDim.x, gx, gyn, gz);
      const Wino4Vec vec = wino4_vectors_load(p_, grp, tn, tid);
      sr = wino4_src<GEO, FORM>(p_, grp, tn, gyn_abs, geo);
      wino4_vectors_store(vec, sVb + (cur ^ 1) * (4 * kBN4), tid);
      nx = Wino4Next{true, tn.kbeg, tn.kcnt};
    }
    wino4_finish<GEO, FORM, SPLIT, w4_epi_mask(EC)>(p, tl, smem, sV, lane, wave, acc, accv, sr, nx);
    prefetched = more;
    cur ^= 1;
    lds_barrier4();
  }
}

struct Wino4Taps { int widx[4][9]; };
constexpr int kRunChunks = 8;
constexpr int kFilterBlocksPerCU = 3;
constexpr int wino4_filter_runs(int kchunks) { return (kchunks + kRunChunks - 1) / kRunChunks; }
__device__ __forceinline__ void wino4_filter_block(const float* __restrict__ w, float* __restrict__ ug, long long unit, int Cin, int Cout, int wrows,
                                                   int wcols, int kchunks, int nvar, const int (&widx)[4][9]) {
  __shared__ float4 sU[kUSlots4];
  __shared__ float4 sG[9 * kBN4];
  const int t256 = (int)threadIdx.x, lane = t256 & 63, wave = t256 >> 6;
  const int nruns = wino4_filter_runs(kchunks);
  const int run = (int)(unit % nruns), var = (int)((unit / nruns) % nvar), ct = (int)(unit / ((long long)nruns * nvar));
  const int kc0 = run * kRunChunks, nch = min(kRunChunks, kchunks - kc0);
  const bool vec = (wcols & 3) == 0 && (reinterpret_cast<uintptr_t>(w) & 15) == 0;
  const int lrow = wave * 8 + (lane >> 3), lch = lane & 7, c0 = (kc0 + lch) * 4;
  float4 gl[2][9];
#pragma unroll
  for (int h = 0; h < 2; ++h) {
    const int oc = ct * kBN4 + h * 32 + lrow;
#pragma unroll
    for (int tp = 0; tp < 9; ++tp) {
      const int wi = widx[var][tp];
      float4 v = make_float4(0.f, 0.f, 0.f, 0.f);
      if (oc < Cout && wi >= 0) {
        const float* src = w + ((size_t)wi * wrows + oc) * wcols + c0;
        if (vec && c0 + 3 < wcols) {
          v = *reinterpret_cast<const float4*>(src);
        } else {
          if (c0 < Cin) v.x = src[0];
          if (c0 + 1 < Cin) v.y = src[1];
          if (c0 + 2 < Cin) v.z = src[2];
          if (c0 + 3 < Cin) v.w = src[3];
        }
        if (c0 >= Cin) v.x = 0.f;
        if (c0 + 1 >= Cin) v.y = 0.f;
        if (c0 + 2 >= Cin) v.z = 0.f;
        if (c0 + 3 >= Cin) v.w = 0.f;
      }
      gl[h][tp] = v;
    }
  }
  const int oc64 = (lane >> 5) * 32 + (lane & 1) * 16 + ((lane >> 1) & 15);
  const double wa = kWa, wb = kWb;
  const double G[6][3] = {{1.0 / kWN0, 0.0, 0.0}, {1.0 / kWNa, wa / kWNa, wa * wa / kWNa}, {1.0 / kWNa, -wa / kWNa, wa * wa / kWNa},
                          {1.0 / kWNb, wb / kWNb, wb * wb / kWNb}, {1.0 / kWNb, -wb / kWNb, wb * wb / kWNb}, {0.0, 0.0, 1.0}};
  float* sUf = reinterpret_cast<float*>(sU);
  float4* dst = reinterpret_cast<float4*>(ug + ((size_t)(ct * nvar + var) * kchunks + kc0) * (kUSlots4 * 4));
  for (int k = 0; k < nch; ++k) {
    if (lch == k) {
#pragma unroll
      for (int h = 0; h < 2; ++h)
#pragma unroll
        for (int tp = 0; tp < 9; ++tp) sG[tp * kBN4 + h * 32 + lrow] = gl[h][tp];
    }
    __syncthreads();
    double g9[3][3];
#pragma unroll
    for (int a = 0; a < 3; ++a)
#pragma unroll
      for (int b = 0; b < 3; ++b) {
        const float4 v = sG[(a * 3 + b) * kBN4 + oc64];
        g9[a][b] = (double)(wave == 0 ? v.x : wave == 1 ? v.y : wave == 2 ? v.z : v.w);
      }
#pragma unroll
    for (int xi = 0; xi < 6; ++xi) {
      double t[3];
#pragma unroll
      for (int b = 0; b < 3; ++b) t[b] = G[xi][0] * g9[0][b] + G[xi][1] * g9[1][b] + G[xi][2] * g9[2][b];
#pragma unroll
      for (int nu = 0; nu < 6; ++nu) sUf[(xi * 6 + nu) * 256 + t256] = (float)(G[nu][0] * t[0] + G[nu][1] * t[1] + G[nu][2] * t[2]);
    }
    __syncthreads();
#pragma unroll
    for (int i = 0; i < kUSlots4 / 256; ++i) dst[(size_t)k * kUSlots4 + i * 256 + t256] = sU[i * 256 + t256];
  }
}
__global__ __launch_bounds__(256, kFilterBlocksPerCU) void wino4_filter_kernel(const IgemmGroup grp, int ngroup, const float* w0, float* u, int Cin, int Cout,
                                                                               int wrows, int wcols, int kchunks, int ntile, int nvar, Wino4Taps tp) {
  const int g = blockIdx.y;
  const float* w = ngroup > 1 ? grp.w[g] : w0;
  wino4_filter_block(w, u + (size_t)g * ntile * nvar * kchunks * (kUSlots4 * 4), blockIdx.x, Cin, Cout, wrows, wcols, kchunks, nvar, tp.widx);
}
__global__ __launch_bounds__(256, kFilterBlocksPerCU) void wino4_filter_batched_kernel(const crdr_w4_filter_item* items, const long long* prefix,
                                                                                       const long long* meta) {
  const int n = (int)meta[0];
  const long long total = meta[1];
  for (long long gu = blockIdx.x; gu < total; gu += gridDim.x) {
    int lo = 0, hi = n - 1;
    while (lo < hi) {
      const int mid = (lo + hi + 1) >> 1;
      if (prefix[mid] <= gu) lo = mid; else hi = mid - 1;
    }
    const crdr_w4_filter_item& it = items[lo];
    const long long ul = gu - prefix[lo];
    const long long per = (long long)it.ntile * it.nvar * wino4_filter_runs(it.kchunks);
    const int g = (int)(ul / per);
    wino4_filter_block(it.w[g], it.u + (size_t)g * it.ntile * it.nvar * it.kchunks * (kUSlots4 * 4), ul - (long long)g * per, it.Cin, it.Cout, it.wrows,
                       it.wcols, it.kchunks, it.nvar, it.widx);
  }
}

}

enum class W4Form { None, K3S1, K5S2, K5S2T, K5S1 };

static W4Form wino4_form(const crdr_conv_desc* d) {
  if (d->wlayout != 0) return W4Form::None;
  if (d->kh == 3 && d->kw == 3 && d->stride == 1) {
    const int grow = d->transposed ? 2 - 2 * d->pad : 2 * d->pad - 2;
    return (d->OH == d->H + grow && d->OW == d->W + grow && d->pad >= 0 && d->pad <= 2) ? W4Form::K3S1 : W4Form::None;
  }
  if (d->kh == 5 && d->kw == 5 && d->stride == 1 && d->pad == 2) return (d->OH == d->H && d->OW == d->W && d->C >= 12) ? W4Form::K5S1 : W4Form::None;
  if (d->kh == 5 && d->kw == 5 && d->stride == 2 && d->pad == 2) {
    if (!d->transposed) return (d->H % 2 == 0 && d->W % 2 == 0 && d->OH == d->H / 2 && d->OW == d->W / 2) ? W4Form::K5S2 : W4Form::None;
    return (d->OH == 2 * d->H && d->OW == 2 * d->W) ? W4Form::K5S2T : W4Form::None;
  }
  return W4Form::None;
}

constexpr size_t kTileSlabBytes = 4 * 2 * 16 * 64 * 16;

struct Wino4Shape {
  W4Form form;
  int geo, gh, gw;
  int tile_rows, tile_cols;
  int GH, GW, patches;
  int ntile, kchunks;
  int nvar, nsub, so;
  long long tiles;
  size_t filter_bytes;
};

static Wino4Shape wino4_shape(const crdr_conv_desc* d, int G) {
  constexpr int kRows[3] = {4 * W4Geo<0>::TY, 4 * W4Geo<1>::TY, 4 * W4Geo<2>::TY}, kCols[3] = {4 * W4Geo<0>::TX, 4 * W4Geo<1>::TX, 4 * W4Geo<2>::TX};
  Wino4Shape s;
  s.form = wino4_form(d);
  const bool phases = s.form == W4Form::K5S2T, stride1 = s.form == W4Form::K3S1 || s.form == W4Form::K5S1;
  const bool pieces = s.form == W4Form::K5S2 || s.form == W4Form::K5S2T || s.form == W4Form::K5S1;
  s.gh = phases ? d->H : d->OH;
  s.gw = phases ? d->W : d->OW;
  s.geo = (stride1 && s.gh <= 16 && s.gw <= 16) ? 2 : (s.gw <= 32 ? 1 : 0);
  s.tile_rows = kRows[s.geo];
  s.tile_cols = kCols[s.geo];
  s.GH = s.geo == 2 ? 1 : cdiv(s.gh, s.tile_rows);
  s.GW = s.geo == 2 ? 1 : cdiv(s.gw, s.tile_cols);
  s.patches = s.geo == 2 ? cdiv(d->N, 2) : d->N * s.GH * s.GW;
  s.ntile = cdiv(d->OC, kBN4);
  s.kchunks = cdiv(d->C, 4);
  s.nvar = pieces ? 4 : 1;
  s.nsub = pieces && !phases ? 4 : 1;
  s.so = phases ? 2 : 1;
  s.tiles = (long long)s.patches * s.ntile * G * (s.so * s.so);
  s.filter_bytes = (size_t)G * s.ntile * s.nvar * s.kchunks * kUSlots4 * 16;
  return s;
}

bool wino4_split_ok(const crdr_conv_desc* d, int G, int nsplit) {
  if (nsplit == 1) return true;
  if (d->flags & CRDR_CONV_NOSPLIT) return false;
  const Wino4Shape sh = wino4_shape(d, G);
  if (sh.form == W4Form::None || nsplit < 1 || nsplit > 16) return false;
  const int Kc = sh.kchunks, K4 = Kc * sh.nsub, cnt = cdiv(K4, nsplit);
  if (K4 - (nsplit - 1) * cnt < 1) return false;
  if (sh.tiles > CRDR_CONV_TICKETS || sh.tiles * nsplit * (long long)kTileSlabBytes >= (1ll << 31)) return false;
  if (sh.form == W4Form::K5S1)
    for (int ks = 1; ks < nsplit; ++ks)
      if ((ks * cnt) % Kc + 3 > Kc && (ks * cnt) % Kc != 0) return false;
  return true;
}

size_t wino4_workspace(const crdr_conv_desc* d, int G, int nsplit) {
  const Wino4Shape sh = wino4_shape(d, G);
  return sh.filter_bytes + (nsplit > 1 ? (size_t)sh.tiles * nsplit * kTileSlabBytes : 0);
}

bool wino4_eligible(const crdr_conv_desc* d, int G, bool vec_ok) {
  const Wino4Shape sh = wino4_shape(d, G);
  if (sh.form == W4Form::None) return false;
  if (d->C % 4 != 0 || d->ldx % 4 != 0 || d->OC % 4 != 0 || d->ldy % 4 != 0) return false;
  if (sh.geo == 2 ? (sh.gh < 9 || sh.gw < 9) : sh.gw < 24) return false;
  if ((d->flags & CRDR_EPI_RES) && d->ldres % 4 != 0) return false;
  if ((d->flags & (CRDR_EPI_RELUMASK | CRDR_EPI_LRELUMASK)) && d->ldmask % 4 != 0) return false;
  if (!wino_admits(d, G) || !vec_ok) return false;
  const long long oimg = (long long)d->N * d->OH * d->OW * std::max(std::max(d->ldy, d->ldres), d->ldmask) * 4;
  if (oimg >= (1ll << 31)) return false;
  if ((long long)sh.filter_bytes / G >= (1ll << 31)) return false;
  return true;
}

int wino4_colsum_rows(const crdr_conv_desc* d) {
  const Wino4Shape sh = wino4_shape(d, 1);
  return sh.patches * sh.so * sh.so;
}

static int wino4_taps(W4Form form, const IgemmTaps& taps, Wino4Taps& wt, int& si) {
  for (int v = 0; v < 4; ++v)
    for (int t = 0; t < 9; ++t) wt.widx[v][t] = -1;
  si = 1;
  if (form == W4Form::K3S1) {
    int dmin;
    if (int rc = tap_window(taps, 3, "Winograd F(4x4)", true, wt.widx[0], &dmin)) return rc;
    si = -dmin;
  } else if (form == W4Form::K5S1) {
    int dmin, win[25];
    if (int rc = tap_window(taps, 5, "Winograd F(4x4)", false, win, &dmin)) return rc;
    for (int dh = 0; dh < 5; ++dh)
      for (int dw = 0; dw < 5; ++dw)
        if (win[dh * 5 + dw] >= 0) wt.widx[(dh / 3) * 2 + dw / 3][(dh % 3) * 3 + dw % 3] = win[dh * 5 + dw];
    si = -dmin;
  } else if (form == W4Form::K5S2) {
    for (int sub = 0; sub < 4; ++sub)
      for (int a2 = 0; a2 < 3; ++a2)
        for (int b2 = 0; b2 < 3; ++b2) {
          const int r = 2 * a2 + (sub >> 1), c = 2 * b2 + (sub & 1);
          if (r < 5 && c < 5) wt.widx[sub][a2 * 3 + b2] = r * 5 + c;
        }
  } else {
    for (int ph = 0; ph < 4; ++ph)
      for (int a2 = 0; a2 < 3; ++a2)
        for (int b2 = 0; b2 < 3; ++b2) {
          const int r = 2 * (2 - a2) + (ph >> 1), c = 2 * (2 - b2) + (ph & 1);
          if (r < 5 && c < 5) wt.widx[ph][a2 * 3 + b2] = r * 5 + c;
        }
  }
  return 0;
}

int wino4_filter_item(const crdr_conv_desc* d, const IgemmTaps& taps, int G, crdr_w4_filter_item* it) {
  CRDR_REQUIRE(wino4_eligible(d, G, true), "conv2d_filter_item: not a convolution the F(4x4, 3x3) kernel takes");
  const Wino4Shape sh = wino4_shape(d, G);
  Wino4Taps wt;
  int si = 1;
  if (int rc = wino4_taps(sh.form, taps, wt, si)) return rc;
  for (int g = 0; g < CRDR_MAX_GROUP; ++g) it->w[g] = nullptr;
  it->u = nullptr;
  it->G = G; it->Cin = d->C; it->Cout = d->OC; it->wrows = d->wrows; it->wcols = d->wcols;
  it->kchunks = sh.kchunks; it->ntile = sh.ntile; it->nvar = sh.nvar;
  for (int v = 0; v < 4; ++v)
    for (int t = 0; t < 9; ++t) it->widx[v][t] = wt.widx[v][t];
  it->units = (long long)G * it->ntile * it->nvar * wino4_filter_runs(it->kchunks);
  return 0;
}

int wino4_filters_batched(const crdr_w4_filter_item* items, const long long* prefix, const long long* meta, hipStream_t s) {
  hipLaunchKernelGGL(wino4_filter_batched_kernel, dim3(kFilterBlocksPerCU * cu_count()), dim3(256), 0, s, items, prefix, meta);
  CRDR_CHECK_LAUNCH("wino4_filter_batched_kernel");
  return 0;
}

static int wino4_transform_filters(const crdr_conv_desc* d, const Wino4Shape& sh, const Wino4Taps& wt, const IgemmGroup& grp, int G, const float* w,
                                   float* u, hipStream_t s) {
  hipLaunchKernelGGL(wino4_filter_kernel, dim3((unsigned)(sh.ntile * sh.nvar * wino4_filter_runs(sh.kchunks)), G), dim3(256), 0, s, grp, G, w, u, d->C,
                     d->OC, d->wrows, d->wcols, sh.kchunks, sh.ntile, sh.nvar, wt);
  CRDR_CHECK_LAUNCH("wino4_filter_kernel");
  return 0;
}

static void wino4_fill_args(IgemmArgs& a, const Wino4Shape& sh, float* u, float* slabs, int nsplit, int si) {
  a.w = u;
  a.nsplit = nsplit;
  a.ws = slabs;
  a.ws_ld = (int)sh.tiles;
  a.nphase = sh.nsub;
  a.kchunks = sh.kchunks * sh.nsub;
  a.so = sh.so;
  a.GH = sh.GH;
  a.GW = sh.GW;
  a.si = si;
  a.cs_rows = sh.patches * sh.so * sh.so;
}

static bool wino4_filter_stationary(const crdr_conv_desc* d, const Wino4Shape& sh, int nsplit, int ncu) {
  const int ksteps = sh.kchunks * sh.nsub;
  const double u_bytes = (double)sh.ntile * sh.so * sh.so * ksteps * (kUSlots4 * 16.0), x_bytes = (double)d->N * d->H * d->W * d->C * 4.0;
  const double ncombo = (double)sh.ntile * sh.so * sh.so, rounds = std::max(1.0, (double)sh.tiles * nsplit / std::max(ncu, 1));
  const double est_patch = x_bytes + 8.0 * u_bytes * (u_bytes > 3.0e6 ? rounds : 1.0), est_fstat = u_bytes + ncombo * x_bytes;
  static const int force_order = [] { const char* e = getenv("CRDR_W4_ORDER"); return e ? atoi(e) : -1; }();
  return force_order >= 0 ? force_order == 1 : est_fstat < est_patch;
}

using Wino4Kern = void (*)(const IgemmArgs, const IgemmGroup, int, int, int);
static Wino4Kern wino4_choose_kernel(int flags, bool split, const Wino4Shape& sh) {
#define W4_ROW(SP, F, E) {wino4_kernel<0, F, SP, E>, wino4_kernel<1, F, SP, E>, wino4_kernel<2, F, SP, E>}
#define W4_CLS(E) {{W4_ROW(false, 0, E), W4_ROW(false, 1, E)}, {W4_ROW(true, 0, E), W4_ROW(true, 1, E)}}
  static const Wino4Kern kerns[4][2][2][3] = {W4_CLS(0), W4_CLS(1), W4_CLS(2), W4_CLS(3)};
#undef W4_CLS
#undef W4_ROW
  static std::atomic<bool> attr_done;
  allow_full_lds(attr_done, &kerns[0][0][0][0], 4 * 2 * 2 * 3);
  return kerns[w4_epi_class(flags)][split ? 1 : 0][sh.form == W4Form::K5S1 ? 1 : 0][sh.geo];
}

int wino4_launch(const crdr_conv_desc* d, IgemmArgs a, const IgemmTaps& taps, const IgemmGroup& grp, int G, float* u, float* slabs, int nsplit,
                 bool filters_ready, hipStream_t s) {
  CRDR_REQUIRE(wino4_eligible(d, G, a.vec_epi != 0), "conv2d: the F(4x4, 3x3) Winograd kernel takes 3x3 / 5x5 stride-1 and 5x5 stride-2 (pad 2) convolutions of >= 24 "
               "output (phase) columns (or whole images of 9..16 pixels a side) with C, OC %% 4 == 0, 16-byte aligned operand rows and no gate / pre-add epilogue");
  const Wino4Shape sh = wino4_shape(d, G);
  Wino4Taps wt;
  int si = 1;
  if (int rc = wino4_taps(sh.form, taps, wt, si)) return rc;
  if (!filters_ready)
    if (int rc = wino4_transform_filters(d, sh, wt, grp, G, a.w, u, s)) return rc;
  wino4_fill_args(a, sh, u, slabs, nsplit, si);
  const int ncu = cu_count();
  const int gyn = wino4_filter_stationary(d, sh, nsplit, ncu) ? -sh.ntile : sh.ntile;
  const Wino4Kern kern = wino4_choose_kernel(a.flags, nsplit > 1, sh);
  const size_t lds = (size_t)(kLdsFloats4 + 2 * 4 * kBN4 + 4) * sizeof(float);
  hipLaunchKernelGGL(kern, dim3(std::min((int)sh.tiles * nsplit, ncu)), dim3(kNT4), lds, s, a, grp, sh.patches, gyn, G);
  CRDR_CHECK_LAUNCH("wino4_kernel");
  return 0;
}

}
```

crdr_amd/hip/ops.py:

```python
from __future__ import annotations

import contextlib
import ctypes as C
import os
from typing import Optional, Tuple

import torch

from . import lib as L
from . import packs, tune
from .batched import BumpArena, JobTable, SiteTables, _capturing, _require_gpu, _stream

_ws_cache = {}
_ws_keep = []
_ws_max = 0

AUTOTUNE = False
FORCED_CONV_ALGO = 0
MATRIX_BF16X3 = False
MATRIX_BF16X6 = False


def _matrix_mode() -> int:
    return 2 if MATRIX_BF16X6 else (1 if MATRIX_BF16X3 else 0)


def _cf() -> int:
    return (0, L.CONV_BF16X3, L.CONV_BF16X6)[_matrix_mode()]


def _wa(algo: int) -> int:
    return int(algo) | (0, L.WGRAD_BF16X3, L.WGRAD_BF16X6)[_matrix_mode()]


def _mk() -> tuple:
    return ((), (1,), (2,))[_matrix_mode()]


_algo_cache, TUNE_LOG, TUNE_REJECTED = tune.algo_cache, tune.LOG, tune.REJECTED
load_tune_cache, save_tune_cache, DEFAULT_TUNE_DB = tune.load, tune.save, tune.DEFAULT_DB

WINOGRAD = os.environ.get("CRDR_WINOGRAD", "1") != "0"
WINO4 = os.environ.get("CRDR_WINO4", "1") != "0"

PREFER_WINOGRAD = False


def _prefer_wino(d, G: int = 1) -> int:
    if not PREFER_WINOGRAD or (d.kh, d.kw, d.stride) not in (((3, 3, 1), (5, 5, 1), (5, 5, 2)) if PREFER_WINOGRAD == 4 else ((3, 3, 1), (5, 5, 1))):
        return 0
    q = L.ConvDesc.from_buffer_copy(d)
    for wid in reversed(tune.ids().wino if PREFER_WINOGRAD == 4 else tune.ids().wino[:2]):
        q.reserved = wid
        if L.load().crdr_conv2d_choose_algo(C.byref(q), G) == wid:
            return wid
    return 0


WINO4_SPLITS = (1, 2, 3, 5, 7, 11, 15)


def _wgrad_wino4_ids():
    w4 = tune.ids().wgrad_wino4
    return [tune.tile_id(w4 - 1, ls) for ls in range(9)] if WINOGRAD and WINO4 and w4 >= 0 else []


RELU_MASK_SINK = None


def _is_wino4(algo: int) -> bool:
    return (algo & 0xFF) == tune.ids().wino4


WINO4_DEMOTED = [0]


def _demote_if_misaligned(d, ios, G: int, explicit: bool) -> None:
    if not explicit and _is_wino4(d.reserved) and any(p_ and int(p_) % 16 for g in range(G) for p_ in (ios[g].y, ios[g].res, ios[g].mask)):
        d.reserved = 0
        WINO4_DEMOTED[0] += 1


def _launch_conv(lib, d, ios, G: int, ws, ws_n, device):
    cached = packs.filter_cache_for(d, ios, G, device) if _is_wino4(d.reserved) else None
    if cached is None:
        return lib.crdr_conv2d_grouped(C.byref(d), ios, G, ws, ws_n, _stream())
    ent, valid = cached
    return lib.crdr_conv2d_grouped_ex(C.byref(d), ios, G, ws, ws_n, ent.u.data_ptr(), ent.nbytes, int(valid), _stream())


_tune_filters = {}


def _conv_workspace(lib, d, G: int, device):
    nb = lib.crdr_conv2d_grouped_workspace(C.byref(d), G)
    return workspace(nb, device, conv=True) if nb else (None, 0)


def _tune_conv_launch(lib, d, ios, G: int, device) -> Tuple[bool, float]:
    w_, wn_ = _conv_workspace(lib, d, G, device)
    nb = int(lib.crdr_conv2d_filter_cache_bytes(C.byref(d), G)) if _is_wino4(d.reserved) else 0
    if not nb or not packs.cacheable(ios, G) or _capturing():
        return lib.crdr_conv2d_grouped(C.byref(d), ios, G, w_, wn_, _stream()) == 0, 0.0
    key = (packs.filter_key(d, ios, G), tuple(packs.version(int(ios[g].w)) for g in range(G)))
    ent = _tune_filters.get(key)
    valid = int(ent is not None and ent.numel() * 4 >= nb)
    if not valid:
        _tune_filters.clear()
        ent = _tune_filters[key] = torch.empty(nb // 4, dtype=torch.float32, device=device)
    return lib.crdr_conv2d_grouped_ex(C.byref(d), ios, G, w_, wn_, ent.data_ptr(), nb, valid, _stream()) == 0, nb / 4.8e9


def _stream_ids():
    ids = list(tune.ids().stream) + (list(tune.ids().wino if WINO4 else tune.ids().wino[:2]) if WINOGRAD else [])
    if WINOGRAD and WINO4 and tune.ids().wino4 >= 0:
        ids += [tune.ids().wino4 | (v << 8) for v in WINO4_SPLITS]
    return ids


def _conv_trial(lib, d, ios, G: int, device, colsum: bool, trial_out):
    if trial_out is not None:
        tio, res_t, reset = ios, trial_out, None
    else:
        span = (d.N * d.OH * d.OW - 1) * d.ldy + d.OC
        res_t, reset = tune.scratch(G * span + 64, device)
        tio = (L.ConvIO * G)()
        C.memmove(tio, ios, C.sizeof(tio))
        for g in range(G):
            tio[g].y = res_t.data_ptr() + 4 * g * span
            if ios[g].pre == ios[g].y:
                tio[g].pre = tio[g].y
            if ios[g].res == ios[g].y:
                tio[g].res = tio[g].y
    keep, cost = [], 0.0

    def run(a):
        nonlocal cost
        d.reserved = a
        if colsum:
            try:
                _, _, nf = _colsum_layout(lib, d, G)
            except L.CrdrHipError:
                return False
            keep[:] = [torch.empty(G * nf, dtype=torch.float32, device=device)]
            for g in range(G):
                tio[g].cs = keep[0].data_ptr() + 4 * g * nf
        ok, cost = _tune_conv_launch(lib, d, tio, G, device)
        return ok
    return run, (lambda: res_t), reset, (lambda: cost)


def _wgrad_trial(lib, d, G: int, pa, qa, device, whole: bool):
    gsize = d.gI * d.gJ * d.kh * d.kw
    tmp = torch.zeros(G * gsize + 64, dtype=torch.float32, device=device)
    ta = (C.c_void_p * G)(*[tmp.data_ptr() + 4 * g * gsize for g in range(G)])
    jobs_t = (L.WgradJob * G)()
    d, slab = L.WgradDesc.from_buffer_copy(d), 0
    d.accumulate = 0 if whole else d.accumulate

    def run(a):
        nonlocal slab
        d.algo = _wa(a)
        nb = lib.crdr_conv2d_wgrad_grouped_workspace(C.byref(d), G)
        if nb == 0 or nb > (2 << 30):
            return False
        slab = nb
        w_, wn_ = workspace(nb, device)
        if whole:
            return lib.crdr_conv2d_wgrad(C.byref(d), pa[0], qa[0], ta[0], w_, wn_, _stream()) == 0
        return lib.crdr_conv2d_wgrad_partial_grouped(C.byref(d), pa, qa, ta, G, w_, wn_, jobs_t, _stream()) == 0
    if whole:
        return run, (lambda: tmp), None, None

    def result():
        reduce_jobs_now(jobs_t, device)
        return tmp
    return run, result, tmp.zero_, (lambda: slab / 3.8e9)


PROFILE = None


def _prof_begin():
    if PROFILE is None:
        return None
    e = torch.cuda.Event(enable_timing=True)
    e.record()
    return e


def _prof_end(kind: str, flops: float, e0, label: str = "", nbytes: float = 0.0) -> None:
    if e0 is None:
        return
    e1 = torch.cuda.Event(enable_timing=True)
    e1.record()
    PROFILE.setdefault(kind, []).append((flops, e0, e1, label, nbytes))


_WS_HEAD = 4 * 16384


def _ws_fit(key, device, need: Optional[int]) -> torch.Tensor:
    size = max(int(_ws_max * 1.25), 1 << 20)
    buf = _ws_cache.get(key)
    if buf is None or buf.numel() < (size if need is None else need):
        if need is not None and torch.cuda.is_current_stream_capturing():
            raise L.CrdrHipError("workspace must be reserved before graph capture (ops.reserve_workspace); "
                                 f"need {need} bytes, have {0 if buf is None else buf.numel()}")
        if buf is not None:
            _ws_keep.append(buf)
        buf = _ws_cache[key] = torch.zeros(size, dtype=torch.uint8, device=device)
    return buf


def workspace(nbytes: int, device, conv: bool = False) -> Tuple[int, int]:
    global _ws_max
    nbytes = int(nbytes) + (0 if conv else _WS_HEAD)
    _ws_max = max(_ws_max, nbytes)
    buf = _ws_fit((device.index if device.index is not None else torch.cuda.current_device(), _stream()), device, nbytes)
    if conv:
        return buf.data_ptr(), buf.numel()
    return buf.data_ptr() + _WS_HEAD, buf.numel() - _WS_HEAD


def reserve_workspace(device, stream: "torch.cuda.Stream") -> None:
    dev = torch.device(device)
    _ws_fit((dev.index if dev.index is not None else torch.cuda.current_device(), stream.cuda_stream), dev, None)


def _pixel_stride(t: torch.Tensor) -> int:
    n, c, h, w = t.shape
    return t.stride(3) if w > 1 else (t.stride(2) if h > 1 else (t.stride(0) if n > 1 else c))


def nhwc(t: torch.Tensor) -> Tuple[torch.Tensor, int]:
    _require_gpu(t)
    n, c, h, w = t.shape
    ld = _pixel_stride(t)
    ok = (c == 1 or t.stride(1) == 1) and ld >= c
    ok = ok and (w == 1 or t.stride(3) == ld) and (h == 1 or t.stride(2) == w * ld) and (n == 1 or t.stride(0) == h * w * ld)
    if not ok or ld % 4 != 0 or (t.data_ptr() % 16) != 0:
        if c % 4 == 0:
            t = t.contiguous(memory_format=torch.channels_last)
            if t.stride(1) != 1 or (w > 1 and t.stride(3) != c):
                t = t.permute(0, 2, 3, 1).contiguous().permute(0, 3, 1, 2)
            ld = c
        else:
            cp = (c + 3) // 4 * 4
            buf = torch.zeros((n, h, w, cp), dtype=t.dtype, device=t.device)
            buf[..., :c] = t.permute(0, 2, 3, 1)
            t = buf.permute(0, 3, 1, 2)[:, :c]
            ld = cp
    return t, ld


def dense_nhwc(t: torch.Tensor) -> torch.Tensor:
    t, ld = nhwc(t)
    if ld != t.shape[1]:
        t = t.permute(0, 2, 3, 1).contiguous().permute(0, 3, 1, 2)
    return t


def ld_for(c: int) -> int:
    return (c + 3) // 4 * 4


def empty_nhwc(n, c, h, w, device, ld: Optional[int] = None, zero: bool = False) -> torch.Tensor:
    ld = ld_for(c) if ld is None else ld
    mk = torch.zeros if (zero or ld != c) else torch.empty
    buf = mk((n, h, w, ld), dtype=torch.float32, device=device)
    return buf.permute(0, 3, 1, 2)[:, :c]


def _p(t: Optional[torch.Tensor]):
    return None if t is None else t.data_ptr()


def round32(v: int) -> int:
    return (v + 31) // 32 * 32


def pack_weight_tapmajor(w: torch.Tensor) -> torch.Tensor:
    _require_gpu(w)
    w = w.contiguous()
    I, J = w.shape[0], w.shape[1]
    T = w.shape[2] * w.shape[3]
    rows, cols = round32(I), round32(4 * T)
    dst = torch.empty((1, rows, cols), dtype=torch.float32, device=w.device)
    lib = L.load()
    L.check(lib.crdr_pack_weight(w.data_ptr(), dst.data_ptr(), I, J, T, rows, cols, 2, _stream()), "pack_weight")
    return dst


def pack_weight(w: torch.Tensor, transpose: bool) -> torch.Tensor:
    _require_gpu(w)
    w = w.contiguous()
    I, J = w.shape[0], w.shape[1]
    T = w.shape[2] * w.shape[3]
    rows, cols = (round32(J), round32(I)) if transpose else (round32(I), round32(J))
    dst = torch.empty((T, rows, cols), dtype=torch.float32, device=w.device)
    lib = L.load()
    L.check(lib.crdr_pack_weight(w.data_ptr(), dst.data_ptr(), I, J, T, rows, cols, int(transpose), _stream()), "pack_weight")
    return dst


_SPAN_LIMIT = (1 << 31) - (1 << 20)


def _colsum_layout(lib, d, G: int):
    rows, ld = C.c_int(), C.c_int()
    L.check(lib.crdr_conv2d_colsum_layout(C.byref(d), G, C.byref(rows), C.byref(ld)), "conv2d_colsum_layout")
    return rows.value, ld.value, max(1, rows.value * 2 * ld.value)


def _conv(lib, d, ios, G: int, key, device, *, flops: float, label: str, nbytes: float, algo: int = 0, plan_as: int = 0,
          colsum: bool = False, trial_out: Optional[torch.Tensor] = None):
    forced = algo or FORCED_CONV_ALGO
    wino = 0 if forced else _prefer_wino(d, G)
    GP = plan_as or G
    if forced or wino:
        d.reserved = forced or wino
    elif AUTOTUNE and key is not None and (GP == G or key in tune.algo_cache):
        algo = tune.algo_cache.get(key)
        if algo is None:
            run, result, reset, penalty = _conv_trial(lib, d, ios, G, device, colsum, trial_out)
            algo = tune.autotune(key, lib.crdr_conv2d_num_configs(), 4, run, extra=_stream_ids(), result=result, reset=reset,
                                 agree=tune.AGREE["conv"], penalty=penalty)
        d.reserved = algo
    elif GP != G:
        d.reserved = lib.crdr_conv2d_choose_algo(C.byref(d), GP)
    _demote_if_misaligned(d, ios, G, bool(forced))
    cs = None
    if colsum:
        rows, ld, nf = _colsum_layout(lib, d, G)
        q = colsum_queue(device)
        cs = [(q.alloc(nf), rows, ld) for _ in range(G)]
        for g in range(G):
            ios[g].cs = cs[g][0]
    ws, ws_n = _conv_workspace(lib, d, G, device)
    e0 = _prof_begin()
    L.check(_launch_conv(lib, d, ios, G, ws, ws_n, device), "conv2d_grouped")
    _prof_end("igemm", flops, e0, label, nbytes)
    return cs


def _wgrad(lib, d, G: int, ps, qs, gs, key, device, *, flops: float, label: str, whole: bool = False, algo: int = 0,
           defer: bool = True) -> list:
    pa, qa, ga = ((C.c_void_p * G)(*v) for v in (ps, qs, gs))
    if algo:
        d.algo = _wa(algo)
    elif AUTOTUNE:
        algo = tune.algo_cache.get(key)
        if algo is None:
            run, result, reset, penalty = _wgrad_trial(lib, d, G, pa, qa, device, whole)
            algo = tune.autotune(key, lib.crdr_conv2d_wgrad_num_configs(), 8, run, extra=_wgrad_wino4_ids(), penalty=penalty, result=result,
                                 reset=reset, agree=tune.AGREE["wgrad"])
        d.algo = _wa(algo)
    nbytes = lib.crdr_conv2d_wgrad_grouped_workspace(C.byref(d), G)
    e0 = _prof_begin()
    queued = []
    if defer:
        assert WGRAD_DEFER is not None, "this launch needs deferred weight-gradient reductions (ops.WGRAD_DEFER)"
        jobs = (L.WgradJob * G)()
        L.check(lib.crdr_conv2d_wgrad_partial_grouped(C.byref(d), pa, qa, ga, G, WGRAD_DEFER.alloc(nbytes), nbytes, jobs, _stream()),
                "conv2d_wgrad_partial_grouped")
        queued = [L.WgradJob.from_buffer_copy(jb) for jb in jobs]
        WGRAD_DEFER.jobs += queued
    else:
        ws, ws_n = workspace(nbytes, device)
        L.check(lib.crdr_conv2d_wgrad(C.byref(d), pa[0], qa[0], ga[0], ws, ws_n, _stream()), "conv2d_wgrad")
    _prof_end("wgrad", flops, e0, label)
    return queued


def conv_out_size(h, k, stride, pad, transposed, out_pad=0):
    if transposed:
        return (h - 1) * stride - 2 * pad + k + out_pad
    return (h + 2 * pad - k) // stride + 1


def conv2d_raw(x: torch.Tensor, wpack: torch.Tensor, oc: int, k: Tuple[int, int], stride: int, pad: int,
               transposed: bool, out_hw: Tuple[int, int], *, bias=None, flags: int = 0, vec2=None, res=None,
               scale=None, shift=None, gate_x=None, gate_t=None, sig_out=None, out: Optional[torch.Tensor] = None,
               algo: int = 0, wlayout: int = 0):
    lib = L.load()
    flags |= _cf()
    x, ldx = nhwc(x)
    n, c, h, w = x.shape
    oh, ow = out_hw
    if out is None:
        out = empty_nhwc(n, oc, oh, ow, x.device)
    out_t, ldy = out, _pixel_stride(out)
    d = L.ConvDesc(N=n, H=h, W=w, C=(c + 3) // 4 * 4 if ldx >= (c + 3) // 4 * 4 else c, OH=oh, OW=ow, OC=oc, kh=k[0], kw=k[1],
                   stride=stride, pad=pad, transposed=int(transposed), ldx=ldx, ldy=ldy, wrows=wpack.shape[1],
                   wcols=wpack.shape[2], flags=flags, ldres=0, ldg=0, wlayout=wlayout, reserved=0)
    io = L.ConvIO(x=x.data_ptr(), w=wpack.data_ptr(), y=out_t.data_ptr(), bias=_p(bias), vec2=_p(vec2))
    if res is not None:
        res, d.ldres = nhwc(res)
        io.res = res.data_ptr()
    if scale is not None:
        io.scale, io.shift = scale.data_ptr(), shift.data_ptr()
    if gate_x is not None:
        gate_x, ldg = nhwc(gate_x)
        gate_t, ldg2 = nhwc(gate_t)
        if ldg != ldg2 or ldg != oc:
            gate_x, gate_t = dense_nhwc(gate_x), dense_nhwc(gate_t)
            ldg = oc
        d.ldg = ldg
        io.gx, io.gt, io.sig = gate_x.data_ptr(), gate_t.data_ptr(), sig_out.data_ptr()
    key = None if flags & L.EPI_ACCUM else ("c", n, h, w, d.C, oh, ow, oc, k, stride, pad, int(transposed), ldx, ldy, flags, d.ldres,
                                            d.ldg, wlayout)
    _conv(lib, d, (L.ConvIO * 1)(io), 1, key, x.device, algo=algo, trial_out=out_t,
          flops=2.0 * n * (h * w if transposed else oh * ow) * c * oc * k[0] * k[1],
          label=f"{'T' if transposed else 'C'} {c}->{oc} k{k[0]}s{stride} in{h}x{w} f{flags}",
          nbytes=4.0 * (n * h * w * c + n * oh * ow * oc * (1 + (res is not None) + 3 * (gate_x is not None)) + k[0] * k[1] * c * oc))
    return out


def conv2d_wgrad_raw(p: torch.Tensor, q: torch.Tensor, g: torch.Tensor, k, stride, pad, accumulate: bool, algo: int = 0,
                      defer: bool = True):
    lib = L.load()
    p, ldp = nhwc(p)
    q, ldq = nhwc(q)
    n, pc, ph, pw = p.shape
    _, qc, qh, qw = q.shape
    if n * ph * pw == 0:
        if not accumulate:
            g.zero_()
        return g
    if n > 1 and max(n * ph * pw * ldp, n * qh * qw * ldq) * 4 >= _SPAN_LIMIT:
        n1 = n // 2
        conv2d_wgrad_raw(p[:n1], q[:n1], g, k, stride, pad, accumulate, algo=algo, defer=False)
        conv2d_wgrad_raw(p[n1:], q[n1:], g, k, stride, pad, True, algo=algo, defer=False)
        return g
    pc4 = min((pc + 3) // 4 * 4, ldp)
    qc4 = min((qc + 3) // 4 * 4, ldq)
    assert g.is_contiguous() and g.shape[0] <= pc4 and g.shape[1] <= qc4
    d = L.WgradDesc(N=n, PH=ph, PW=pw, PC=pc4, ldp=ldp, QH=qh, QW=qw, QC=qc4, ldq=ldq, kh=k[0], kw=k[1],
                    stride=stride, pad=pad, gI=g.shape[0], gJ=g.shape[1], accumulate=int(accumulate), algo=_wa(0))
    key = ("w", n, ph, pw, pc4, ldp, qh, qw, qc4, ldq, k, stride, pad, g.shape[0], g.shape[1]) + _mk()
    _wgrad(lib, d, 1, [p.data_ptr()], [q.data_ptr()], [g.data_ptr()], key, p.device, whole=True, algo=algo,
           defer=defer and WGRAD_DEFER is not None and WGRAD_DEFER.device == p.device,
           flops=2.0 * n * ph * pw * g.shape[0] * g.shape[1] * k[0] * k[1], label=f"W {g.shape[0]}x{g.shape[1]} k{k[0]}s{stride} p{ph}x{pw}")
    return g


class DeferredWgrad:
    CAP = 4096

    def __init__(self, device, arena_bytes: int = 2 << 30):
        self.device = torch.device(device)
        self._arena = BumpArena(self.device, arena_bytes, "DeferredWgrad: arena")
        self.alloc = self._arena.alloc
        self.jobs = []
        self.tables = SiteTables(self.device, L.WgradJob, self.CAP, name="DeferredWgrad")

    def pending(self) -> int:
        return len(self.jobs)

    def drop(self) -> None:
        self.jobs = []
        self._arena.rewind()

    def flush(self, key=None) -> None:
        if not self.jobs:
            return
        rounds = []
        for jb in self.jobs:
            for r in rounds:
                if jb.g not in r[1]:
                    r[0].append(jb); r[1].add(jb.g)
                    break
            else:
                rounds.append(([jb], {jb.g}))
        for ri, (js, _) in enumerate(rounds):
            tb = self.tables.upload((key, ri), js, _wgrad_job_tiles)
            L.check(L.load().crdr_wgrad_reduce_batched(*tb.operands, _stream()), "wgrad_reduce_batched")
        self.jobs = []
        self._arena.reset()


def _wgrad_job_tiles(j) -> int:
    return (j.gI * j.gJ * j.T + 255) // 256 if (j.smallj or j.T > 32) else j.gI * ((j.gJ + 63) // 64)


def reduce_jobs_now(jobs, device) -> None:
    tb = JobTable(device, L.WgradJob, len(jobs), name="reduce_jobs_now").upload(jobs, _wgrad_job_tiles)
    L.check(L.load().crdr_wgrad_reduce_batched(*tb.operands, _stream()), "wgrad_reduce_batched")
    torch.cuda.current_stream().synchronize()


WGRAD_DEFER: Optional[DeferredWgrad] = None


_local_defers = {}


@contextlib.contextmanager
def local_wgrad_defer(device, site):
    global WGRAD_DEFER
    prev = WGRAD_DEFER
    if prev is not None and prev.device == device:
        yield
        return
    d = _local_defers.get(device)
    if d is None:
        d = _local_defers[device] = DeferredWgrad(device, arena_bytes=256 << 20)
    WGRAD_DEFER = d
    try:
        yield
        d.flush(site)
    except BaseException:
        d.drop()
        raise
    finally:
        WGRAD_DEFER = prev


def flush_wgrads(key=None) -> None:
    if WGRAD_DEFER is not None:
        WGRAD_DEFER.flush(key)


def pending_wgrads() -> int:
    return WGRAD_DEFER.pending() if WGRAD_DEFER is not None else 0


def colsum(x: torch.Tensor, out: torch.Tensor, accumulate: bool):
    lib = L.load()
    x, ld = nhwc(x)
    n, c, h, w = x.shape
    m = n * h * w
    nbytes = lib.crdr_colsum_workspace(m, c)
    ws, ws_n = workspace(nbytes, x.device)
    L.check(lib.crdr_colsum(x.data_ptr(), ld, m, c, out.data_ptr(), int(accumulate), ws, ws_n, _stream()), "colsum")
    return out


def epilogue_bwd(dout, out, flags, *, vec2=None, scale=None, shift=None, gate_t=None, sig=None, need_dz=True,
                 dbias_accum: Optional[torch.Tensor] = None):
    lib = L.load()
    dout, lddout = nhwc(dout)
    n, c, h, w = dout.shape
    m = n * h * w
    d = L.EbwdDesc(M=m, C=c, flags=flags, lddout=lddout, ldout=0, lddz=ld_for(c), ldgres=ld_for(c), ldg=c)
    io = L.EbwdIO(dout=dout.data_ptr(), vec2=_p(vec2), scale=_p(scale), shift=_p(shift))
    if out is not None:
        out, d.ldout = nhwc(out)
        io.out = out.data_ptr()
    dz = gres = dgt = None
    if need_dz:
        dz = empty_nhwc(n, c, h, w, dout.device)
        io.dz = dz.data_ptr()
    if flags & L.EPI_GATE:
        gate_t, ldg = nhwc(gate_t)
        sig, ldg2 = nhwc(sig)
        assert ldg == c and ldg2 == c
        io.gt, io.sig = gate_t.data_ptr(), sig.data_ptr()
        gres = empty_nhwc(n, c, h, w, dout.device)
        dgt = empty_nhwc(n, c, h, w, dout.device)
        io.gres, io.dgt = gres.data_ptr(), dgt.data_ptr()
    elif (flags & L.EPI_AFFINE) and (flags & L.EPI_RES):
        gres = empty_nhwc(n, c, h, w, dout.device)
        io.gres = gres.data_ptr()
    colsums = torch.empty((4, c), dtype=torch.float32, device=dout.device)
    io.colsums = colsums.data_ptr()
    if dbias_accum is not None:
        assert dbias_accum.is_contiguous() and dbias_accum.numel() == c
        io.dbias_accum = dbias_accum.data_ptr()
    nbytes = lib.crdr_epilogue_bwd_workspace(C.byref(d))
    ws, ws_n = workspace(nbytes, dout.device)
    L.check(lib.crdr_epilogue_bwd(C.byref(d), C.byref(io), ws, ws_n, _stream()), "epilogue_bwd")
    return dz, gres, dgt, colsums


class V:
    __slots__ = ("ptr", "ld", "c")

    def __init__(self, ptr: int, ld: int, c: int):
        self.ptr, self.ld, self.c = ptr, ld, c


def view(buf: torch.Tensor, c0: int, c: int) -> V:
    return V(buf.data_ptr() + 4 * c0, buf.shape[-1], c)


def _conv_ios(xs, wpacks, ys, biases=None, pres=None, masks=None, ress=None, vec2=None, scale=None, shift=None):
    ios = (L.ConvIO * len(xs))()
    for g, io in enumerate(ios):
        io.x, io.w, io.y, io.vec2 = xs[g].ptr, wpacks[g], ys[g].ptr, vec2
        if biases is not None:
            io.bias = biases[g]
        if pres is not None:
            io.pre = pres[g].ptr
        if masks is not None:
            io.mask = masks[g].ptr
        if ress is not None:
            io.res = ress[g].ptr
        if scale is not None:
            io.scale, io.shift = scale, shift
    return ios


def conv_group(n: int, h: int, w: int, xs, wpacks, ys, oc: int, k: Tuple[int, int], pad: int, transposed: bool, *,
               wrows: int, wcols: int, biases=None, pres=None, masks=None, flags: int = 0, device=None, label: str = "",
               plan_as: Optional[int] = None):
    lib = L.load()
    G = len(xs)
    x0, y0 = xs[0], ys[0]
    if biases is not None:
        flags |= L.EPI_BIAS
    if pres is not None:
        flags |= L.EPI_PREADD
    if masks is not None:
        flags |= L.EPI_RELUMASK
    self_res = flags == L.EPI_ACCUM
    if self_res:
        flags = L.EPI_RES
    flags |= _cf()
    d = L.ConvDesc(N=n, H=h, W=w, C=x0.c, OH=h, OW=w, OC=oc, kh=k[0], kw=k[1], stride=1, pad=pad, transposed=int(transposed),
                   ldx=x0.ld, ldy=y0.ld, wrows=wrows, wcols=wcols, flags=flags, ldres=y0.ld if self_res else 0, ldg=0, wlayout=0, reserved=0,
                   ldpre=pres[0].ld if pres is not None else 0, ldmask=masks[0].ld if masks is not None else 0)
    ios = _conv_ios(xs, wpacks, ys, biases, pres, masks, ys if self_res else None)
    GP = plan_as or G
    key = ("g", GP, n, h, w, d.C, oc, k, pad, int(transposed), d.ldx, d.ldy, flags, d.ldpre, d.ldmask, wrows, wcols)
    _conv(lib, d, ios, G, key, device, plan_as=GP,
          flops=2.0 * G * n * h * w * x0.c * oc * k[0] * k[1],
          label=f"{'T' if transposed else 'C'} {G}x {x0.c}->{oc} k{k[0]} in{h}x{w} f{flags} {label}",
          nbytes=4.0 * G * (n * h * w * x0.c + n * h * w * oc * (1 + (pres is not None) + (masks is not None) + bool(flags & L.EPI_ACCUM))
                            + k[0] * k[1] * x0.c * oc))


def wgrad_group(n: int, h: int, w: int, ps, qs, gs, gi: int, gj: int, k: Tuple[int, int], pad: int, *, device, accumulate=True,
                label: str = ""):
    lib = L.load()
    G = len(ps)
    p0, q0 = ps[0], qs[0]
    d = L.WgradDesc(N=n, PH=h, PW=w, PC=p0.c, ldp=p0.ld, QH=h, QW=w, QC=q0.c, ldq=q0.ld, kh=k[0], kw=k[1], stride=1, pad=pad,
                    gI=gi, gJ=gj, accumulate=int(accumulate), algo=_wa(0))
    key = ("wg", G, n, h, w, p0.c, p0.ld, q0.c, q0.ld, k, pad, gi, gj) + _mk()
    jobs = _wgrad(lib, d, G, [v.ptr for v in ps], [v.ptr for v in qs], [g[0] for g in gs], key, device,
                  flops=2.0 * G * n * h * w * gi * gj * k[0] * k[1], label=f"W {G}x {gi}x{gj} k{k[0]} p{h}x{w} {label}")
    for jb, g in zip(jobs, gs):
        jb.gJtot = g[1]


def wgrad_split(n: int, h: int, w: int, p: V, q: V, parts, k: Tuple[int, int], pad: int, *, device, label: str = ""):
    lib = L.load()
    d = L.WgradDesc(N=n, PH=h, PW=w, PC=p.c, ldp=p.ld, QH=h, QW=w, QC=q.c, ldq=q.ld, kh=k[0], kw=k[1], stride=1, pad=pad,
                    gI=p.c, gJ=q.c, accumulate=1, algo=_wa(0))
    key = ("ws", n, h, w, p.c, p.ld, q.c, q.ld, k, pad) + _mk()
    job, = _wgrad(lib, d, 1, [p.ptr], [q.ptr], [parts[0][2]], key, device, whole=True,
                  flops=2.0 * n * h * w * p.c * q.c * k[0] * k[1], label=f"W {p.c}x{q.c} k{k[0]} p{h}x{w} {label}")
    split = []
    for row0, rows, gptr, gjtot in parts:
        jb = L.WgradJob.from_buffer_copy(job)
        jb.slab = job.slab + 4 * row0 * q.c
        jb.g, jb.gI, jb.gJtot = gptr, rows, gjtot
        split.append(jb)
    WGRAD_DEFER.jobs[-1:] = split


def colsum_scatter(x: V, m: int, block: int, outs_table: torch.Tensor, device, accumulate: bool = True):
    lib = L.load()
    nbytes = lib.crdr_colsum_workspace(m, x.c)
    ws, ws_n = workspace(nbytes, device)
    L.check(lib.crdr_colsum_scatter(x.ptr, x.ld, m, x.c, block, outs_table.data_ptr(), int(accumulate), ws, ws_n, _stream()),
            "colsum_scatter")


class ColsumQueue:
    CAP = 512

    def __init__(self, device, arena_bytes: int = 128 << 20):
        self.device = torch.device(device)
        self._arena = BumpArena(self.device, arena_bytes, "ColsumQueue: arena")
        self._scratch = BumpArena(self.device, 16 << 20, "ColsumQueue: scratch")
        self.scratch_off = 0
        self.jobs = []
        self.tables = SiteTables(self.device, L.ColsumJob, self.CAP, rows=2, name="ColsumQueue")

    arena = property(lambda self: self._arena.tensor)

    def alloc(self, nfloats: int) -> int:
        return self._arena.alloc(4 * nfloats)

    def add(self, cs_ptr: int, rows: int, ld: int, c: int, out_pre: Optional[int], out_post: Optional[int], accumulate: bool):
        slab = L.load().crdr_colsum_slab_rows()
        nslab, cpad = (rows + slab - 1) // slab, (c + 63) // 64 * 64
        off = self.scratch_off
        self.scratch_off += nslab * 2 * cpad
        self.jobs.append(L.ColsumJob(cs=cs_ptr, out_pre=out_pre, out_post=out_post, rows=rows, ld=ld, C=c, accumulate=int(accumulate),
                                     nslab=nslab, cpad=cpad, scratch_off=off))

    def drop(self) -> None:
        self.jobs, self.scratch_off = [], 0
        self._arena.rewind()

    def flush(self, key) -> None:
        if self.jobs:
            scratch = self._scratch.reserve(4 * self.scratch_off)
            tb = self.tables.upload(key, self.jobs, lambda j: ((j.cpad // 64) * j.nslab, j.cpad // 64),
                                    trailer=scratch.to_bytes(8, "little"))
            L.check(L.load().crdr_colsum_finish_batched(*tb.operands, scratch, _stream()), "colsum_finish_batched")
        self.jobs, self.scratch_off = [], 0
        self._arena.reset()
        self._scratch.reset()


_colsum_queues = {}


def colsum_queue(device) -> ColsumQueue:
    dev = torch.device(device)
    dev = torch.device("cuda", torch.cuda.current_device()) if dev.index is None else dev
    q = _colsum_queues.get(dev)
    if q is None:
        q = _colsum_queues[dev] = ColsumQueue(dev)
    return q


def conv_multi(n: int, h: int, w: int, oh: int, ow: int, xs, wpacks, ys, oc: int, k: Tuple[int, int], stride: int, pad: int,
               transposed: bool, *, wrows: int, wcols: int, biases=None, pres=None, masks=None, ress=None, vec2=None, scale=None,
               shift=None, flags: int = 0, colsum: bool = False, wlayout: int = 0, device=None, label: str = ""):
    lib = L.load()
    G = len(xs)
    x0, y0 = xs[0], ys[0]
    if biases is not None:
        flags |= L.EPI_BIAS
    if pres is not None:
        flags |= L.EPI_PREADD
    if ress is not None:
        flags |= L.EPI_RES
    if scale is not None:
        flags |= L.EPI_AFFINE
    if colsum:
        flags |= L.EPI_COLSUM
    flags |= _cf()
    cin = min((x0.c + 3) // 4 * 4, x0.ld)
    d = L.ConvDesc(N=n, H=h, W=w, C=cin, OH=oh, OW=ow, OC=oc, kh=k[0], kw=k[1], stride=stride, pad=pad, transposed=int(transposed),
                   ldx=x0.ld, ldy=y0.ld, wrows=wrows, wcols=wcols, flags=flags, ldres=ress[0].ld if ress is not None else 0, ldg=0,
                   wlayout=wlayout, reserved=0, ldpre=pres[0].ld if pres is not None else 0,
                   ldmask=masks[0].ld if masks is not None else 0)
    ios = _conv_ios(xs, wpacks, ys, biases, pres, masks, ress, vec2, scale, shift)
    key = ("m", G, n, h, w, oh, ow, d.C, oc, k, stride, pad, int(transposed), d.ldx, d.ldy, flags, d.ldres, d.ldpre, d.ldmask,
           wrows, wcols, wlayout)
    return _conv(lib, d, ios, G, key, device, colsum=colsum,
                 flops=2.0 * G * n * (h * w if transposed else oh * ow) * x0.c * oc * k[0] * k[1],
                 label=f"{'T' if transposed else 'C'} {G}x {x0.c}->{oc} k{k[0]}s{stride} in{h}x{w} f{flags} {label}",
                 nbytes=4.0 * G * (n * h * w * x0.c + n * oh * ow * oc * (1 + (pres is not None) + (masks is not None) + (ress is not None)
                                                                          + bool(flags & L.EPI_ACCUM)) + k[0] * k[1] * x0.c * oc))


def wgrad_multi(n: int, ph: int, pw: int, qh: int, qw: int, ps, qs, gs, gi: int, gj: int, k: Tuple[int, int], stride: int, pad: int, *,
                device, label: str = ""):
    lib = L.load()
    G = len(ps)
    p0, q0 = ps[0], qs[0]
    pc, qc = min((p0.c + 3) // 4 * 4, p0.ld), min((q0.c + 3) // 4 * 4, q0.ld)
    d = L.WgradDesc(N=n, PH=ph, PW=pw, PC=pc, ldp=p0.ld, QH=qh, QW=qw, QC=qc, ldq=q0.ld, kh=k[0], kw=k[1], stride=stride, pad=pad,
                    gI=gi, gJ=gj, accumulate=1, algo=_wa(0))
    key = ("wm", G, n, ph, pw, pc, p0.ld, qh, qw, qc, q0.ld, k, stride, pad, gi, gj) + _mk()
    _wgrad(lib, d, G, [v.ptr for v in ps], [v.ptr for v in qs], gs, key, device,
           flops=2.0 * G * n * ph * pw * gi * gj * k[0] * k[1], label=f"W {G}x {gi}x{gj} k{k[0]}s{stride} p{ph}x{pw} {label}")
```

Baseline: 225.6 img/s.

## Add pair-tile F(4x4,3x3) Winograd variant that packs two patches' channel tails

Adds a pair-tile mode to the F(4x4,3x3) Winograd kernel, selected by id bit 12. When the output channel count leaves a tail of 1..32 columns in the last 64-wide block, two adjacent spatial patches share one tile for that tail, halving filter LDS per patch and doubling raw input buffers. This removes wasted MFMA work on padded output channels and cuts the tile count. The autotuner adds these ids as candidates for such shapes. The cost is more kernel instantiations, extra tile-index arithmetic, and an added barrier after each tile in pair mode.

```diff
diff --git a/crdr_amd/csrc/algo_id.hpp b/crdr_amd/csrc/algo_id.hpp
--- a/crdr_amd/csrc/algo_id.hpp
+++ b/crdr_amd/csrc/algo_id.hpp
@@ -2,6 +2,7 @@
 
 namespace crdr {
 
+constexpr int kAlgoPairBit = 1 << 12;
 enum AlgoFamily { kAlgoBuiltIn, kAlgoTiled , kAlgoStream, kAlgoWino2, kAlgoWino4, kAlgoBeyond  };
 struct AlgoId {
   AlgoFamily family;
@@ -18,6 +19,7 @@
 inline AlgoId conv_algo_decode(int reserved, int ntiled, int nstream) { return algo_decode(reserved, {ntiled, nstream, 2, 1}); }
 inline AlgoId wgrad_algo_decode(int algo, int ndirect) { return algo_decode(algo & 0xffff, {ndirect, 0, 1, 1}); }
 
+inline bool conv_algo_pairs(int reserved) { return (reserved & kAlgoPairBit) != 0; }
 inline int conv_algo_splits(const AlgoId& id) { return id.family == kAlgoWino4 ? id.split + 1 : 1 << id.split; }
 inline int wgrad_algo_splits(const AlgoId& id) { return 1 << id.split; }
 
diff --git a/crdr_amd/csrc/api.cpp b/crdr_amd/csrc/api.cpp
--- a/crdr_amd/csrc/api.cpp
+++ b/crdr_amd/csrc/api.cpp
@@ -65,5 +65,5 @@
 }
 
 extern "C" const char* crdr_last_error(void) { return crdr::g_err; }
-extern "C" int crdr_version(void) { return 600; }
+extern "C" int crdr_version(void) { return 601; }
 extern "C" const char* crdr_arch(void) { return "gfx950"; }
diff --git a/crdr_amd/csrc/igemm.hip b/crdr_amd/csrc/igemm.hip
--- a/crdr_amd/csrc/igemm.hip
+++ b/crdr_amd/csrc/igemm.hip
@@ -269,6 +269,7 @@
     CRDR_REQUIRE(!fallback && wino4_eligible(d, G, true), "conv2d: forced F(4x4, 3x3) Winograd kernel: not a 3x3 / 5x5 stride-1 or 5x5 stride-2 convolution it takes (wino4_eligible)");
     nsplit = conv_algo_splits(id);
     CRDR_REQUIRE(wino4_split_ok(d, G, nsplit), "conv2d: F(4x4, 3x3) Winograd kernel: %d K splits do not fit this shape", nsplit);
+    CRDR_REQUIRE(!conv_algo_pairs(d->reserved) || wino4_pairs_ok(d, G), "conv2d: F(4x4, 3x3) pair tiles (id bit 12): needs a 3x3 stride-1 convolution of more than 16 x 16 pixels and a channel tail OC %% 64 of 1..32");
   } else {
     CRDR_REQUIRE(!fallback && wino_eligible(d, G), "conv2d: forced Winograd kernel: not a 3x3 / 5x5 stride-1 convolution it takes");
     CRDR_REQUIRE(id.index == 0 || wino_pairs_ok(d), "conv2d: Winograd pair-tile variant: needs a channel tail of 1..32 and more than one patch");
@@ -396,6 +397,7 @@
 static int build_plan(const crdr_conv_desc* d, Plan* pl, int G = 1, bool fallback = false) {
   if (int rc = plan_geometry(d, pl, G)) return rc;
   const AlgoId id = conv_algo_decode(d->reserved, kNumCfgs, stream_num_variants());
+  CRDR_REQUIRE(!conv_algo_pairs(d->reserved) || id.family == kAlgoWino4, "conv2d: id bit 12 (pair tiles) belongs to the F(4x4, 3x3) Winograd kernel");
   if (id.family == kAlgoWino2 || id.family == kAlgoWino4) return plan_wino(d, pl, G, id, fallback);
   int sv = id.family == kAlgoStream ? id.index : -1;
   if (id.family == kAlgoBuiltIn && !fallback) sv = choose_stream(d, pl->a, G);
@@ -432,7 +434,7 @@
   const bool f4 = pl.wino == WinoKernel::F4, f2 = pl.wino == WinoKernel::F2 || pl.wino == WinoKernel::F2Pairs;
   const AlgoFamily family = f4 ? kAlgoWino4 : (f2 ? kAlgoWino2 : (pl.stream >= 0 ? kAlgoStream : kAlgoTiled));
   const int index = f4 ? 0 : (f2 ? (pl.wino == WinoKernel::F2Pairs ? 1 : 0) : (pl.stream >= 0 ? pl.stream : pl.cfg));
-  return conv_algo_encode(family, index, pl.a.nsplit, kNumCfgs, stream_num_variants());
+  return conv_algo_encode(family, index, pl.a.nsplit, kNumCfgs, stream_num_variants()) | (f4 && conv_algo_pairs(d->reserved) ? kAlgoPairBit : 0);
 }
 
 extern "C" double crdr_conv2d_flops(const crdr_conv_desc* d) {
diff --git a/crdr_amd/csrc/wino.hpp b/crdr_amd/csrc/wino.hpp
--- a/crdr_amd/csrc/wino.hpp
+++ b/crdr_amd/csrc/wino.hpp
@@ -37,6 +37,7 @@
 bool wino4_eligible(const crdr_conv_desc* d, int G, bool vec_ok);
 size_t wino4_workspace(const crdr_conv_desc* d, int G, int nsplit);
 bool wino4_split_ok(const crdr_conv_desc* d, int G, int nsplit);
+bool wino4_pairs_ok(const crdr_conv_desc* d, int G);
 int wino4_colsum_rows(const crdr_conv_desc* d);
 int wino4_filter_item(const crdr_conv_desc* d, const IgemmTaps& taps, int G, crdr_w4_filter_item* it);
 int wino4_filters_batched(const crdr_w4_filter_item* items, const long long* prefix, const long long* meta, hipStream_t s);
diff --git a/crdr_amd/csrc/wino4.hip b/crdr_amd/csrc/wino4.hip
--- a/crdr_amd/csrc/wino4.hip
+++ b/crdr_amd/csrc/wino4.hip
@@ -1,6 +1,7 @@
 #include <algorithm>
 #include <type_traits>
 
+#include "algo_id.hpp"
 #include "common.hpp"
 #include "igemm_args.hpp"
 #include "wino.hpp"
@@ -27,6 +28,12 @@
 constexpr int kRawBufs = 3, kFiltBufs = 3;
 constexpr int kRF = kInSlots4 * 4, kFF = kUSlots4 * 4;
 constexpr int kLdsFloats4 = kRawBufs * kRF + kFiltBufs * kFF;
+constexpr int kRFP = 2 * kRF, kFFP = kFF / 2;
+constexpr int kPairFilt = kRawBufs * kRFP;
+constexpr int kPairSink = kPairFilt + kFiltBufs * kFFP;
+constexpr int kPairColsum = kPairFilt + 2 * kFFP;
+static_assert(kPairSink + 2 * 256 <= kLdsFloats4, "a pair tile fits the LDS of a full one");
+static_assert(kPairColsum >= kRawBufs * kRF + 2 * kFF && kPairColsum + 4096 <= kPairSink, "column sums: clear of F0, F1 and the sink of either layout");
 
 __device__ __forceinline__ void lds_barrier4() {
   __builtin_amdgcn_sched_barrier(0);
@@ -44,15 +51,33 @@
   o3 = pk_fma(pk_bc(kWb3), w, pk_bc(kWa3) * q) + m5;
 }
 
-struct Wino4Tile { int gidx, n, oh0, ow0, n0, patch, tn, phase, lin, ks, kbeg, kcnt; };
+struct Wino4Tile { int gidx, n, oh0, ow0, n0, patch, tn, phase, lin, ks, kbeg, kcnt, pair; };
 
 template <int GEO>
+__device__ __forceinline__ void wino4_patch_at(const IgemmArgs& p, int patch, int& n, int& oh0, int& ow0) {
+  const int ppi = p.GH * p.GW;
+  n = patch / ppi;
+  const int prem = patch - n * ppi, by = prem / p.GW, bx = prem - by * p.GW;
+  oh0 = by * (4 * W4Geo<GEO>::TY);
+  ow0 = bx * (4 * W4Geo<GEO>::TX);
+}
+template <int GEO>
+__device__ __forceinline__ Wino4Tile wino4_pair_side(const IgemmArgs& p, const Wino4Tile& tl, int oh) {
+  Wino4Tile t = tl;
+  t.patch = tl.patch + oh;
+  wino4_patch_at<GEO>(p, t.patch, t.n, t.oh0, t.ow0);
+  return t;
+}
+
+template <bool PAIR> __device__ __forceinline__ int wino4_items(int gx, int gyn, int nph) { return PAIR ? gx * (gyn - 1) + ((gx + 1) >> 1) : gx * gyn * nph; }
+
+template <int GEO, bool PAIR = false>
 __device__ __forceinline__ Wino4Tile wino4_tile(const IgemmArgs& p, int vb, int gx, int gyn_, int gz) {
   const bool fstat = gyn_ < 0;
   const int gyn = fstat ? -gyn_ : gyn_;
   Wino4Tile t;
   const int nph = p.so * p.so;
-  const int T = gx * gyn * nph, S = p.nsplit, nwg = T * gz * S, cpx = nwg >> 3;
+  const int T = wino4_items<PAIR>(gx, gyn, nph), S = p.nsplit, nwg = T * gz * S, cpx = nwg >> 3;
   const int qs = vb < cpx * 8 ? (vb & 7) * cpx + (vb >> 3) : vb;
   const int q = qs / S;
   t.ks = qs - q * S;
@@ -65,7 +90,32 @@
   t.gidx = q / T;
   const int r = q - t.gidx * T;
   int tn;
-  if (fstat) {
+  t.pair = 0;
+  if constexpr (PAIR) {
+    const int nfull = gyn - 1;
+    t.phase = 0;
+    if (fstat) {
+      if (r < nfull * gx) {
+        tn = r / gx;
+        t.patch = r - tn * gx;
+      } else {
+        tn = nfull;
+        t.patch = 2 * (r - nfull * gx);
+        t.pair = 1;
+      }
+    } else {
+      const int U = 2 * nfull + 1, u = r / U, w = r - u * U, nf = min(2, gx - 2 * u) * nfull;
+      if (w < nf) {
+        const int second = w >= nfull ? 1 : 0;
+        t.patch = 2 * u + second;
+        tn = w - second * nfull;
+      } else {
+        tn = nfull;
+        t.patch = 2 * u;
+        t.pair = 1;
+      }
+    }
+  } else if (fstat) {
     const int combo = r / gx;
     t.patch = r - combo * gx;
     tn = combo / nph;
@@ -82,11 +132,7 @@
     t.oh0 = 0;
     t.ow0 = 0;
   } else {
-    const int ppi = p.GH * p.GW;
-    t.n = t.patch / ppi;
-    const int prem = t.patch - t.n * ppi, by = prem / p.GW, bx = prem - by * p.GW;
-    t.oh0 = by * (4 * W4Geo<GEO>::TY);
-    t.ow0 = bx * (4 * W4Geo<GEO>::TX);
+    wino4_patch_at<GEO>(p, t.patch, t.n, t.oh0, t.ow0);
   }
   t.n0 = tn * kBN4;
   return t;
@@ -115,17 +161,18 @@
   return ok ? (unsigned)((((n * p.H + ih) * p.W + iw) * p.ldx) * 4) : kOobOffset;
 }
 
-struct Wino4Src {
+template <bool PAIR = false> struct Wino4Src {
   __amdgpu_buffer_rsrc_t rx, ru;
   unsigned u_off0;
-  unsigned a_off[4];
+  unsigned a_off[PAIR ? 8 : 4];
 };
 
 __device__ __forceinline__ __amdgpu_buffer_rsrc_t wino4_empty_rsrc() { return __builtin_amdgcn_make_buffer_rsrc(nullptr, 0, 0, 0x00020000); }
 
-__device__ __forceinline__ void wino4_dma_raw(float* smem, const Wino4Src& sr, __amdgpu_buffer_rsrc_t rx, int j, int soff, int rbuf, int lane, int wave) {
+template <bool PAIR, bool PT = false>
+__device__ __forceinline__ void wino4_dma_raw(float* smem, const Wino4Src<PAIR>& sr, __amdgpu_buffer_rsrc_t rx, int j, int soff, int rbuf, int lane, int wave) {
   const int piece = wave + 4 * j;
-  __builtin_amdgcn_raw_ptr_buffer_load_lds(rx, (lds_ptr_t)(smem + rbuf * kRF + piece * 256), 16, (int)sr.a_off[j], soff, 0, 0);
+  __builtin_amdgcn_raw_ptr_buffer_load_lds(rx, (lds_ptr_t)(smem + rbuf * (PT ? kRFP : kRF) + piece * 256), 16, (int)sr.a_off[j], soff, 0, 0);
 }
 template <int FORM>
 __device__ __forceinline__ int wino4_raw_soff(const IgemmArgs& p, int kr) {
@@ -134,15 +181,31 @@
   if (FORM == 1) return ch * 16;
   return ch * 16 + ((sub >> 1) * p.W + (sub & 1)) * p.ldx * 4;
 }
-__device__ __forceinline__ void wino4_dma_filt(float* smem, const Wino4Src& sr, __amdgpu_buffer_rsrc_t ru, int j, int kf, int fbuf, int lane, int wave) {
+template <bool PAIR>
+__device__ __forceinline__ void wino4_dma_filt(float* smem, const Wino4Src<PAIR>& sr, __amdgpu_buffer_rsrc_t ru, int j, int kf, int fbuf, int lane, int wave) {
   const int piece = wave * 9 + j;
   const unsigned so = (unsigned)__builtin_amdgcn_readfirstlane((int)sr.u_off0) + (unsigned)kf * (kUSlots4 * 16u) + (unsigned)piece * 1024u;
   __builtin_amdgcn_raw_ptr_buffer_load_lds(ru, (lds_ptr_t)(smem + kRawBufs * kRF + fbuf * kFF + piece * 256), 16, lane * 16, (int)so, 0, 0);
 }
-constexpr int kW4PrologueReqs = 30;
-template <int FORM>
-__device__ __forceinline__ void wino4_prologue_req(const IgemmArgs& p, float* smem, const Wino4Src& sr, int kbeg, int kcnt, int lane, int wave, int i) {
-  if (i < 12) {
+__device__ __forceinline__ void wino4_dma_filt_pair(float* smem, const Wino4Src<true>& sr, __amdgpu_buffer_rsrc_t ru, int j, int kf, int fbuf, int lane, int wave) {
+  const bool sink = j == 4 && wave >= 2;
+  const int piece = 4 * wave + min(wave, 2) + j;
+  const unsigned so = (unsigned)__builtin_amdgcn_readfirstlane((int)sr.u_off0) + (unsigned)kf * (kUSlots4 * 16u) + (unsigned)piece * 2048u;
+  float* dst = sink ? smem + kPairSink + (wave - 2) * 256 : smem + kPairFilt + fbuf * kFFP + piece * 256;
+  __builtin_amdgcn_raw_ptr_buffer_load_lds(sink ? wino4_empty_rsrc() : ru, (lds_ptr_t)dst, 16, (lane >> 3) * 256 + (lane & 7) * 16, (int)so, 0, 0);
+}
+template <bool PT> constexpr int w4_prologue_reqs() { return PT ? 3 * 8 + 2 * 5 : 3 * 4 + 2 * 9; }
+template <int FORM, bool PAIR, bool PT = false>
+__device__ __forceinline__ void wino4_prologue_req(const IgemmArgs& p, float* smem, const Wino4Src<PAIR>& sr, int kbeg, int kcnt, int lane, int wave, int i) {
+  if constexpr (PT) {
+    if (i < 24) {
+      const int kr = i >> 3;
+      wino4_dma_raw<PAIR, true>(smem, sr, kr < kcnt ? sr.rx : wino4_empty_rsrc(), i & 7, wino4_raw_soff<FORM>(p, kbeg + kr), kr, lane, wave);
+    } else {
+      const int kf = (i - 24) / 5;
+      wino4_dma_filt_pair(smem, sr, kf < kcnt ? sr.ru : wino4_empty_rsrc(), (i - 24) - 5 * kf, kbeg + kf, kf, lane, wave);
+    }
+  } else if (i < 12) {
     const int kr = i >> 2;
     wino4_dma_raw(smem, sr, kr < kcnt ? sr.rx : wino4_empty_rsrc(), i & 3, wino4_raw_soff<FORM>(p, kbeg + kr), kr, lane, wave);
   } else {
@@ -150,21 +213,22 @@
     wino4_dma_filt(smem, sr, kf < kcnt ? sr.ru : wino4_empty_rsrc(), (i - 12) - 9 * kf, kbeg + kf, kf, lane, wave);
   }
 }
-template <int FORM>
-__device__ __forceinline__ void wino4_prologue_dma(const IgemmArgs& p, float* smem, const Wino4Src& sr, int kbeg, int kcnt, int lane, int wave) {
-#pragma unroll
-  for (int i = 0; i < kW4PrologueReqs; ++i) wino4_prologue_req<FORM>(p, smem, sr, kbeg, kcnt, lane, wave, i);
-}
-struct Wino4Next { bool more; int kbeg, kcnt; };
-
-template <int GEO, int FORM>
-__device__ __forceinline__ void wino4_loop(const IgemmArgs& p, const Wino4Tile& tl, float* smem, Wino4Src& sr, bool prefetched, int lane, int wave,
+template <int FORM, bool PAIR, bool PT = false>
+__device__ __forceinline__ void wino4_prologue_dma(const IgemmArgs& p, float* smem, const Wino4Src<PAIR>& sr, int kbeg, int kcnt, int lane, int wave) {
+#pragma unroll
+  for (int i = 0; i < w4_prologue_reqs<PT>(); ++i) wino4_prologue_req<FORM, PAIR, PT>(p, smem, sr, kbeg, kcnt, lane, wave, i);
+}
+struct Wino4Next { bool more; int kbeg, kcnt, pair; };
+
+template <int GEO, int FORM, bool PAIR, bool PT>
+__device__ __forceinline__ void wino4_loop(const IgemmArgs& p, const Wino4Tile& tl, float* smem, Wino4Src<PAIR>& sr, bool prefetched, int lane, int wave,
                                            f32x4 (&acc)[64], f32x4 (&accv)[8], const unsigned (&geo)[4]) {
+  constexpr int RS = PT ? kRFP : kRF, FS = PT ? kFFP : kFF, PS = PT ? 128 : 256, NFQ = PT ? 5 : 9;
   const int K4 = tl.kcnt, kbeg = tl.kbeg;
   const int tx = lane & 15, kg = lane >> 4, th = wave >> 1, oh = wave & 1;
-  const int rbase = (w4_slot0<GEO>(th) + w4_ty<GEO>(th, tx) * W4Geo<GEO>::PR + w4_tx<GEO>(tx)) * 4 + kg;
+  const int rbase = (w4_slot0<GEO>(th) + w4_ty<GEO>(th, tx) * W4Geo<GEO>::PR + w4_tx<GEO>(tx)) * 4 + kg + (PT ? oh * kRF : 0);
   auto ro = [](int i, int j) constexpr { return (((i & 3) * 4 + (j & 3)) * kClsSlots + (i >> 2) * W4Geo<GEO>::PR + (j >> 2)) * 4; };
-  const int fbase = kRawBufs * kRF + kg * kBN4 + 32 * oh + 2 * tx;
+  const int fbase = PT ? kPairFilt + kg * 32 + 2 * tx : kRawBufs * kRF + kg * kBN4 + 32 * oh + 2 * tx;
 
   const W4Consts kc = w4_consts();
   f32x2v T[6][3];
@@ -183,7 +247,7 @@
   auto hpass = [&](int x) __attribute__((always_inline)) { bt6_row(T[x][0], T[x][1], T[x][2], V[x], kc); };
 
   if (!prefetched) {
-    wino4_prologue_dma<FORM>(p, smem, sr, kbeg, K4, lane, wave);
+    wino4_prologue_dma<FORM, PAIR, PT>(p, smem, sr, kbeg, K4, lane, wave);
     __builtin_amdgcn_s_waitcnt(0x0070);
   } else {
     __builtin_amdgcn_s_waitcnt(0x8070);
@@ -204,7 +268,7 @@
   float uf[9][2];
 #pragma unroll
   for (int j = 0; j < 4; ++j) {
-    const f32x2 u2 = *reinterpret_cast<const f32x2*>(smem + fbase + j * 256);
+    const f32x2 u2 = *reinterpret_cast<const f32x2*>(smem + fbase + j * PS);
     uf[j][0] = u2[0];
     uf[j][1] = u2[1];
   }
@@ -224,9 +288,9 @@
   };
   auto sub_state = [&](int k, int r0_, int r1_, int ch3_, int sub3_) __attribute__((always_inline)) {
     SubState st;
-    st.rpo = rbase + r1_ * kRF;
-    st.fpo = fbase + r0_ * kFF;
-    st.fpno = fbase + r1_ * kFF;
+    st.rpo = rbase + r1_ * RS;
+    st.fpo = fbase + r0_ * FS;
+    st.fpno = fbase + r1_ * FS;
     asm volatile("" : "+v"(st.rpo));
     asm volatile("" : "+v"(st.fpo));
     asm volatile("" : "+v"(st.fpno));
@@ -252,7 +316,7 @@
       if (s < 64) acc[s] = __builtin_amdgcn_mfma_f32_16x16x4f32(uf[j % 9][ob], v_elem(V[x], y), acc[s], 0, 0, 0);
       else asm volatile("v_mfma_f32_16x16x4_f32 %0, %1, %2, %0" : "+v"(accv[s - 64]) : "v"(uf[j % 9][ob]), "v"(v_elem(V[x], y)));
       if (ob == 1 && j + 4 < 36) {
-        const f32x2 u2 = *reinterpret_cast<const f32x2*>(fp + (j + 4) * 256);
+        const f32x2 u2 = *reinterpret_cast<const f32x2*>(fp + (j + 4) * PS);
         uf[(j + 4) % 9][0] = u2[0];
         uf[(j + 4) % 9][1] = u2[1];
       }
@@ -267,15 +331,20 @@
         nxt = sub_state(k + 1, r0, r1, ch3, sub3);
       }
       if (s >= 66 && s < 70) {
-        const f32x2 u2 = *reinterpret_cast<const f32x2*>(fpn + (s - 66) * 256);
+        const f32x2 u2 = *reinterpret_cast<const f32x2*>(fpn + (s - 66) * PS);
         uf[s - 66][0] = u2[0];
         uf[s - 66][1] = u2[1];
       }
       if (ob == 0 && s < 36) vread(rp, s >> 1);
       if (ob == 0 && s >= 36 && s <= 60) {
         const int q = (s - 36) >> 1;
-        if (q < 9) wino4_dma_filt(smem, sr, ru2, q, kbeg + k + 2, f2, lane, wave);
-        else wino4_dma_raw(smem, sr, rx3, q - 9, soff3, r0, lane, wave);
+        if constexpr (PT) {
+          if (q < NFQ) wino4_dma_filt_pair(smem, sr, ru2, q, kbeg + k + 2, f2, lane, wave);
+          else wino4_dma_raw<PAIR, true>(smem, sr, rx3, q - NFQ, soff3, r0, lane, wave);
+        } else {
+          if (q < 9) wino4_dma_filt(smem, sr, ru2, q, kbeg + k + 2, f2, lane, wave);
+          else wino4_dma_raw(smem, sr, rx3, q - 9, soff3, r0, lane, wave);
+        }
       }
       __builtin_amdgcn_sched_barrier(0);
       if (s == 15) vpass(0);
@@ -319,13 +388,19 @@
   return (f & ~w4_epi_mask(0)) == 0 ? 0 : (f & ~w4_epi_mask(1)) == 0 ? 1 : (f & ~w4_epi_mask(2)) == 0 ? 2 : 3;
 }
 
-template <int GEO, int FORM, bool SPLIT, int FM>
-__device__ __forceinline__ void wino4_finish(const IgemmArgs& p, const Wino4Tile& tl, float* smem, const float* sV, int lane, int wave, f32x4 (&acc)[64],
-                                             f32x4 (&accv)[8], const Wino4Src& srn, const Wino4Next nx) {
+template <int GEO, int FORM, bool SPLIT, int FM, bool PAIR>
+__device__ __forceinline__ void wino4_finish(const IgemmArgs& p, const Wino4Tile& tl_, float* smem, const float* sV, int lane, int wave, f32x4 (&acc)[64],
+                                             f32x4 (&accv)[8], const Wino4Src<PAIR>& srn, const Wino4Next nx) {
+  const bool pt = PAIR && tl_.pair != 0;
+  Wino4Tile tl = tl_;
+  if constexpr (PAIR) {
+    if (pt && (wave & 1)) tl = wino4_pair_side<GEO>(p, tl_, 1);
+  }
+  const bool side_live = !pt || tl.patch < p.N * p.GH * p.GW;
   const int f = p.flags & FM;
   const bool has_res = (f & CRDR_EPI_RES) != 0, has_mask = (f & (CRDR_EPI_RELUMASK | CRDR_EPI_LRELUMASK)) != 0;
   const bool do_cs = (f & CRDR_EPI_COLSUM) != 0, accum = (f & CRDR_EPI_ACCUM) != 0;
-  const int tx = lane & 15, kg = lane >> 4, th = wave >> 1, oh = wave & 1;
+  const int tx = lane & 15, kg = lane >> 4, th = wave >> 1, oh = pt ? 0 : (wave & 1);
   const int oy0 = tl.oh0 + 4 * w4_ty<GEO>(th, tx), ox0 = tl.ow0 + 4 * w4_tx<GEO>(tx);
   auto tdesc = [&](const float* base, int ld) __attribute__((always_inline)) {
     const unsigned long long bytes = (((unsigned long long)p.N * p.OH * p.OW - 1) * ld + p.Cout) * 4ull;
@@ -341,12 +416,22 @@
 #pragma unroll
     for (int b = 0; b < 4; ++b) pixm |= (img < p.N && so * (oy0 + a) + py < p.OH && so * (ox0 + b) + px < p.OW) ? (1u << (4 * a + b)) : 0u;
   auto soff = [&](int ld, int a, int b) __attribute__((always_inline)) { return so * (a * p.OW + b) * ld * 4; };
-  float* sC = smem + kRawBufs * kRF + 2 * kFF;
+  float* sC = smem + (PAIR ? kPairColsum : kRawBufs * kRF + 2 * kFF);
 
   auto next_reqs = [&](int grp) __attribute__((always_inline)) {
     __builtin_amdgcn_sched_barrier(0);
-#pragma unroll
-    for (int i = (3 * grp) / 2; i < (3 * (grp + 1)) / 2; ++i) wino4_prologue_req<FORM>(p, smem, srn, nx.kbeg, nx.kcnt, lane, wave, i);
+    if constexpr (PAIR) {
+      if (nx.pair) {
+#pragma unroll
+        for (int i = (34 * grp) / 20; i < (34 * (grp + 1)) / 20; ++i) wino4_prologue_req<FORM, PAIR, true>(p, smem, srn, nx.kbeg, nx.kcnt, lane, wave, i);
+      } else {
+#pragma unroll
+        for (int i = (3 * grp) / 2; i < (3 * (grp + 1)) / 2; ++i) wino4_prologue_req<FORM>(p, smem, srn, nx.kbeg, nx.kcnt, lane, wave, i);
+      }
+    } else {
+#pragma unroll
+      for (int i = (3 * grp) / 2; i < (3 * (grp + 1)) / 2; ++i) wino4_prologue_req<FORM>(p, smem, srn, nx.kbeg, nx.kcnt, lane, wave, i);
+    }
     __builtin_amdgcn_sched_barrier(0);
   };
   auto out_transform = [&](int ob, float (&yv)[4][4][4], auto reqs_c) __attribute__((always_inline)) {
@@ -387,7 +472,10 @@
   unsigned slab_bytes = 0;
   auto slab_off = [&](int ob, int q) __attribute__((always_inline)) { return (unsigned)((((wave * 2 + ob) * 16 + q) * 64 + lane) * 16); };
   if constexpr (SPLIT) {
-    if (nx.more) wino4_prologue_dma<FORM>(p, smem, srn, nx.kbeg, nx.kcnt, lane, wave);
+    if (nx.more) {
+      if (PAIR && nx.pair) wino4_prologue_dma<FORM, PAIR, PAIR>(p, smem, srn, nx.kbeg, nx.kcnt, lane, wave);
+      else wino4_prologue_dma<FORM>(p, smem, srn, nx.kbeg, nx.kcnt, lane, wave);
+    }
     constexpr unsigned kTileSlab = 4u * 2u * 16u * 64u * 16u;
     slab_bytes = (unsigned)p.ws_ld * kTileSlab;
     rws = __builtin_amdgcn_make_buffer_rsrc(p.ws + (size_t)tl.lin * (kTileSlab / 4), 0, 0x7fffffff, 0x00020000);
@@ -398,7 +486,7 @@
 #pragma unroll
       for (int q = 0; q < 16; ++q) {
         const f32x4 v = {yv[q >> 2][q & 3][0], yv[q >> 2][q & 3][1], yv[q >> 2][q & 3][2], yv[q >> 2][q & 3][3]};
-        __builtin_amdgcn_raw_buffer_store_b128(__builtin_bit_cast(u32x4_t, v), rws, slab_off(ob, q) + (unsigned)tl.ks * slab_bytes, 0, 16 );
+        __builtin_amdgcn_raw_buffer_store_b128(__builtin_bit_cast(u32x4_t, v), rws, side_live ? slab_off(ob, q) + (unsigned)tl.ks * slab_bytes : kOobOffset, 0, 16 );
       }
     }
     asm volatile("s_waitcnt vmcnt(0)" ::: "memory");
@@ -458,7 +546,7 @@
           f32x4 l[4];
 #pragma unroll
           for (int j = 0; j < 4; ++j)
-            l[j] = __builtin_bit_cast(f32x4, __builtin_amdgcn_raw_buffer_load_b128(rws, s0 + j < p.nsplit ? slab_off(ob, q) + (unsigned)(s0 + j) * slab_bytes : kOobOffset, 0, 16));
+            l[j] = __builtin_bit_cast(f32x4, __builtin_amdgcn_raw_buffer_load_b128(rws, s0 + j < p.nsplit && side_live ? slab_off(ob, q) + (unsigned)(s0 + j) * slab_bytes : kOobOffset, 0, 16));
 #pragma unroll
           for (int j = 0; j < 4; ++j) v += l[j];
         }
@@ -561,14 +649,16 @@
       float sum = 0.f;
       for (int th2 = 0; th2 < 2; ++th2)
         for (int t2 = 0; t2 < 16; ++t2) sum += sC[((((th2 * 2 + oh2) * 2 + which) * 2 + ob2) * 64 + kg2 * 16 + t2) * 4 + r];
-      if (tl.n0 + c < p.Cout) p.cs[(((size_t)tl.patch * (p.so * p.so) + tl.phase) * 2 + which) * p.cs_ld + tl.n0 + c] = sum;
-    }
-  }
-}
-
-template <int GEO, int FORM>
-__device__ __forceinline__ Wino4Src wino4_src(const IgemmArgs& p, const IgemmGroup& grp, const Wino4Tile& tl, int gyn, const unsigned (&geo)[4]) {
-  Wino4Src sr;
+      if (pt) {
+        if (tl_.n0 + (c & 31) < p.Cout && tl_.patch + oh2 < p.N * p.GH * p.GW) p.cs[((size_t)(tl_.patch + oh2) * 2 + which) * p.cs_ld + tl_.n0 + (c & 31)] = sum;
+      } else if (tl.n0 + c < p.Cout) p.cs[(((size_t)tl.patch * (p.so * p.so) + tl.phase) * 2 + which) * p.cs_ld + tl.n0 + c] = sum;
+    }
+  }
+}
+
+template <int GEO, int FORM, bool PAIR>
+__device__ __forceinline__ Wino4Src<PAIR> wino4_src(const IgemmArgs& p, const IgemmGroup& grp, const Wino4Tile& tl, int gyn, const unsigned (&geo)[4]) {
+  Wino4Src<PAIR> sr;
   const float* x = p.ngroup > 1 ? grp.x[tl.gidx] : p.x;
   sr.rx = __builtin_amdgcn_make_buffer_rsrc(const_cast<float*>(x), 0, (unsigned)((((unsigned long long)p.N * p.H * p.W - 1) * p.ldx + p.Cin) * 4ull), 0x00020000);
   const int nph = p.so * p.so;
@@ -578,6 +668,11 @@
   const int sub0 = FORM == 1 ? tl.kbeg / (p.kchunks / p.nphase) : 0;
 #pragma unroll
   for (int j = 0; j < 4; ++j) sr.a_off[j] = wino4_in_off<GEO, FORM>(p, tl, geo[j], sub0);
+  if constexpr (PAIR) {
+    const Wino4Tile tb = wino4_pair_side<GEO>(p, tl, 1);
+#pragma unroll
+    for (int j = 0; j < 4; ++j) sr.a_off[4 + j] = tl.pair ? wino4_in_off<GEO, FORM>(p, tb, geo[j], sub0) : kOobOffset;
+  }
   return sr;
 }
 
@@ -604,16 +699,16 @@
   }
 }
 
-template <int GEO, int FORM, bool SPLIT, int EC>
+template <int GEO, int FORM, bool SPLIT, int EC, bool PAIR = false>
 __global__ __launch_bounds__(kNT4) void wino4_kernel(const IgemmArgs p_, const IgemmGroup grp, int gx, int gyn, int gz) {
   extern __shared__ __attribute__((aligned(16))) float smem[];
   const int lane_ = threadIdx.x & 63, wave_ = __builtin_amdgcn_readfirstlane(threadIdx.x >> 6);
   const int gyn_abs = gyn < 0 ? -gyn : gyn;
-  const int total = gx * gyn_abs * gz * p_.so * p_.so * (SPLIT ? p_.nsplit : 1);
+  const int total = PAIR ? wino4_items<PAIR>(gx, gyn_abs, 1) * gz * (SPLIT ? p_.nsplit : 1) : gx * gyn_abs * gz * p_.so * p_.so * (SPLIT ? p_.nsplit : 1);
   float* sVb = smem + kLdsFloats4;
   int cur = 0;
   bool prefetched = false;
-  Wino4Src sr;
+  Wino4Src<PAIR> sr;
   unsigned geo[4];
 #pragma unroll
   for (int j = 0; j < 4; ++j) geo[j] = wino4_piece_geo<GEO>(wave_ + 4 * j, lane_);
@@ -622,7 +717,7 @@
     asm volatile("" : "+v"(lane));
     asm volatile("" : "+s"(wave));
     const int tid = wave * 64 + lane;
-    const Wino4Tile tl = wino4_tile<GEO>(p_, vb, gx, gyn, gz);
+    const Wino4Tile tl = wino4_tile<GEO, PAIR>(p_, vb, gx, gyn, gz);
     IgemmArgs p = p_;
     if (p.ngroup > 1) {
       const int g = tl.gidx;
@@ -631,7 +726,7 @@
     float* sV = sVb + cur * (4 * kBN4);
     if (!prefetched) {
       const Wino4Vec vec = wino4_vectors_load(p_, grp, tl, tid);
-      sr = wino4_src<GEO, FORM>(p_, grp, tl, gyn_abs, geo);
+      sr = wino4_src<GEO, FORM, PAIR>(p_, grp, tl, gyn_abs, geo);
       wino4_vectors_store(vec, sV, tid);
     }
     f32x4 acc[64], accv[8];
@@ -639,17 +734,26 @@
     for (int j = 0; j < 64; ++j) acc[j] = f32x4{0.f, 0.f, 0.f, 0.f};
 #pragma unroll
     for (int j = 0; j < 8; ++j) accv[j] = f32x4{0.f, 0.f, 0.f, 0.f};
-    wino4_loop<GEO, FORM>(p, tl, smem, sr, prefetched, lane, wave, acc, accv, geo);
+    if constexpr (PAIR) {
+      if (tl.pair) wino4_loop<GEO, FORM, true, true>(p, tl, smem, sr, prefetched, lane, wave, acc, accv, geo);
+      else wino4_loop<GEO, FORM, true, false>(p, tl, smem, sr, prefetched, lane, wave, acc, accv, geo);
+    } else {
+      wino4_loop<GEO, FORM, false, false>(p, tl, smem, sr, prefetched, lane, wave, acc, accv, geo);
+    }
+    if constexpr (PAIR) {
+      __builtin_amdgcn_s_waitcnt(0x0070);
+      lds_barrier4();
+    }
     const bool more = vb + (int)gridDim.x < total;
     Wino4Next nx{false, 0, 0};
     if (more) {
-      const Wino4Tile tn = wino4_tile<GEO>(p_, vb + (int)gridDim.x, gx, gyn, gz);
+      const Wino4Tile tn = wino4_tile<GEO, PAIR>(p_, vb + (int)gridDim.x, gx, gyn, gz);
       const Wino4Vec vec = wino4_vectors_load(p_, grp, tn, tid);
-      sr = wino4_src<GEO, FORM>(p_, grp, tn, gyn_abs, geo);
+      sr = wino4_src<GEO, FORM, PAIR>(p_, grp, tn, gyn_abs, geo);
       wino4_vectors_store(vec, sVb + (cur ^ 1) * (4 * kBN4), tid);
-      nx = Wino4Next{true, tn.kbeg, tn.kcnt};
-    }
-    wino4_finish<GEO, FORM, SPLIT, w4_epi_mask(EC)>(p, tl, smem, sV, lane, wave, acc, accv, sr, nx);
+      nx = Wino4Next{true, tn.kbeg, tn.kcnt, tn.pair};
+    }
+    wino4_finish<GEO, FORM, SPLIT, w4_epi_mask(EC), PAIR>(p, tl, smem, sV, lane, wave, acc, accv, sr, nx);
     prefetched = more;
     cur ^= 1;
     lds_barrier4();
@@ -782,6 +886,7 @@
   int tile_rows, tile_cols;
   int GH, GW, patches;
   int ntile, kchunks;
+  bool pair;
   int nvar, nsub, so;
   long long tiles;
   size_t filter_bytes;
@@ -802,13 +907,20 @@
   s.GW = s.geo == 2 ? 1 : cdiv(s.gw, s.tile_cols);
   s.patches = s.geo == 2 ? cdiv(d->N, 2) : d->N * s.GH * s.GW;
   s.ntile = cdiv(d->OC, kBN4);
+  s.pair = conv_algo_pairs(d->reserved);
   s.kchunks = cdiv(d->C, 4);
   s.nvar = pieces ? 4 : 1;
   s.nsub = pieces && !phases ? 4 : 1;
   s.so = phases ? 2 : 1;
-  s.tiles = (long long)s.patches * s.ntile * G * (s.so * s.so);
+  s.tiles = s.pair ? ((long long)s.patches * (s.ntile - 1) + cdiv(s.patches, 2)) * G : (long long)s.patches * s.ntile * G * (s.so * s.so);
   s.filter_bytes = (size_t)G * s.ntile * s.nvar * s.kchunks * kUSlots4 * 16;
   return s;
+}
+
+bool wino4_pairs_ok(const crdr_conv_desc* d, int G) {
+  const Wino4Shape sh = wino4_shape(d, G);
+  const int tail = d->OC % kBN4;
+  return sh.form == W4Form::K3S1 && sh.geo != 2 && tail >= 1 && tail <= 32;
 }
 
 bool wino4_split_ok(const crdr_conv_desc* d, int G, int nsplit) {
@@ -937,6 +1049,15 @@
 
 using Wino4Kern = void (*)(const IgemmArgs, const IgemmGroup, int, int, int);
 static Wino4Kern wino4_choose_kernel(int flags, bool split, const Wino4Shape& sh) {
+  if (sh.pair) {
+#define W4_PAIR(SP, E) {wino4_kernel<0, 0, SP, E, true>, wino4_kernel<1, 0, SP, E, true>}
+    static const Wino4Kern pairs[4][2][2] = {{W4_PAIR(false, 0), W4_PAIR(true, 0)}, {W4_PAIR(false, 1), W4_PAIR(true, 1)},
+                                             {W4_PAIR(false, 2), W4_PAIR(true, 2)}, {W4_PAIR(false, 3), W4_PAIR(true, 3)}};
+#undef W4_PAIR
+    static std::atomic<bool> pair_attr_done;
+    allow_full_lds(pair_attr_done, &pairs[0][0][0], 4 * 2 * 2);
+    return pairs[w4_epi_class(flags)][split ? 1 : 0][sh.geo];
+  }
 #define W4_ROW(SP, F, E) {wino4_kernel<0, F, SP, E>, wino4_kernel<1, F, SP, E>, wino4_kernel<2, F, SP, E>}
 #define W4_CLS(E) {{W4_ROW(false, 0, E), W4_ROW(false, 1, E)}, {W4_ROW(true, 0, E), W4_ROW(true, 1, E)}}
   static const Wino4Kern kerns[4][2][2][3] = {W4_CLS(0), W4_CLS(1), W4_CLS(2), W4_CLS(3)};
@@ -952,6 +1073,7 @@
   CRDR_REQUIRE(wino4_eligible(d, G, a.vec_epi != 0), "conv2d: the F(4x4, 3x3) Winograd kernel takes 3x3 / 5x5 stride-1 and 5x5 stride-2 (pad 2) convolutions of >= 24 "
                "output (phase) columns (or whole images of 9..16 pixels a side) with C, OC %% 4 == 0, 16-byte aligned operand rows and no gate / pre-add epilogue");
   const Wino4Shape sh = wino4_shape(d, G);
+  CRDR_REQUIRE(!sh.pair || wino4_pairs_ok(d, G), "conv2d: F(4x4, 3x3) pair tiles (id bit 12) take a 3x3 stride-1 convolution of more than 16 x 16 pixels with OC %% 64 in 1..32");
   Wino4Taps wt;
   int si = 1;
   if (int rc = wino4_taps(sh.form, taps, wt, si)) return rc;
diff --git a/crdr_amd/hip/ops.py b/crdr_amd/hip/ops.py
--- a/crdr_amd/hip/ops.py
+++ b/crdr_amd/hip/ops.py
@@ -111,10 +111,15 @@
     return lib.crdr_conv2d_grouped_ex(C.byref(d), ios, G, w_, wn_, ent.data_ptr(), nb, valid, _stream()) == 0, nb / 4.8e9
 
 
-def _stream_ids():
+WINO4_PAIRS = 0x1000
+
+
+def _stream_ids(oc: int = 0):
     ids = list(tune.ids().stream) + (list(tune.ids().wino if WINO4 else tune.ids().wino[:2]) if WINOGRAD else [])
     if WINOGRAD and WINO4 and tune.ids().wino4 >= 0:
         ids += [tune.ids().wino4 | (v << 8) for v in WINO4_SPLITS]
+        if 0 < oc % 64 <= 32:
+            ids += [tune.ids().wino4 | WINO4_PAIRS | (v << 8) for v in (0,) + WINO4_SPLITS]
     return ids
 
 
@@ -324,7 +329,7 @@
         algo = tune.algo_cache.get(key)
         if algo is None:
             run, result, reset, penalty = _conv_trial(lib, d, ios, G, device, colsum, trial_out)
-            algo = tune.autotune(key, lib.crdr_conv2d_num_configs(), 4, run, extra=_stream_ids(), result=result, reset=reset,
+            algo = tune.autotune(key, lib.crdr_conv2d_num_configs(), 4, run, extra=_stream_ids(d.OC), result=result, reset=reset,
                                  agree=tune.AGREE["conv"], penalty=penalty)
         d.reserved = algo
     elif GP != G:
```

After: 227.1 img/s, median of 6. No clear change (+0.7%).
